# goroda/c3sc

Measured on AMD Instinct MI355X. Metric: Bellman-sweep nodes/sec (7D car rank-10), higher is better.
Workload: dtype f64

## Files before the change

### c3sc_amd/csrc/c3sc_hip.hip

```cpp
#include <hip/hip_runtime.h>

#include <algorithm>
#include <cmath>
#include <cstdio>
#include <cstdlib>
#include <cstring>
#include <string>
#include <vector>

#include "../../include/c3sc_hip.h"
#include "fiber_partition.hpp"
#include "kernel_common.hpp"
#include "kernel_rollout.hpp"
#include "kernel_rollout_ode.hpp"
#include "model_tables.hpp"
#include "registry.hpp"

namespace c3sc {

std::vector<KernelEntry> &kernel_registry()
{
    static std::vector<KernelEntry> reg;
    return reg;
}
// ... 715 lines not shown
    const int d = c->d;
    std::vector<int> rps(nstack);
    std::vector<long> offs((size_t)nstack * MAXD, 0);
    size_t off = c->static_doubles;
    for (int s = 0; s < nstack; s++) {
        const size_t *r = ranks + (size_t)s * (d + 1);
        if (r[0] != 1 || r[d] != 1) return fail(c, C3SC_ERR_ARG, "upload_value_stack: ranks[s][0] and ranks[s][d] must be 1");
        size_t maxrank = 1;
        for (int m = 0; m <= d; m++) {
            if (r[m] < 1) return fail(c, C3SC_ERR_ARG, "upload_value_stack: rank < 1");
            maxrank = std::max(maxrank, r[m]);
        }
        for (int m = 0; m < d; m++)
            if (!cores[(size_t)s * d + m]) return fail(c, C3SC_ERR_ARG, "upload_value_stack: null core");
        rps[s] = pick_rp(d, (int)maxrank, c->model, C3SC_VARIANT_AUTO);
        if (rps[s] == 0) return fail(c, C3SC_ERR_UNSUPPORTED, "upload_value_stack: no kernel instantiation for a stage's (dim, rank)");
        for (int m = 0; m < d; m++) {
            offs[(size_t)s * MAXD + m] = (long)off;
            const size_t per = (m == 0 || m == d - 1) ? rps[s] : (size_t)rps[s] * rps[s];
            off += ((size_t)c->ngrid[m] * per + 15) & ~(size_t)15;
        }
    }
    std::vector<double> buf(off - c->static_doubles, 0.0);
    for (int s = 0; s < nstack; s++) {
        double *dst[MAXD];
        for (int m = 0; m < d; m++) dst[m] = buf.data() + (offs[(size_t)s * MAXD + m] - (long)c->static_doubles);
        pad_cores_host(d, c->ngrid, rps[s], ranks + (size_t)s * (d + 1), cores + (size_t)s * d, dst);
    }
    HIPCHK(c, hipSetDevice(c->device));
    if (c->hz_stack) HIPCHK(c, hipFree(c->hz_stack));
    c->hz_stack = nullptr;
    c->hz_nstack = 0;
    HIPCHK(c, hipMalloc((void **)&c->hz_stack, off * sizeof(double)));
    HIPCHK(c, hipMemcpy(c->hz_stack + c->static_doubles, buf.data(), buf.size() * sizeof(double), hipMemcpyHostToDevice));
    c->hz_stack_static = c->static_doubles;
    c->hz_rp.swap(rps);
    c->hz_core_off.swap(offs);
    c->hz_nstack = nstack;
    return C3SC_OK;
}

int c3sc_hip_upload_value_device(c3sc_hip_ctx *c, const size_t *ranks, const double *const *d_cores, void *stream)
{
    size_t cd = 0;
    int rc = prepare_value(c, ranks, &cd);
    if (rc != C3SC_OK) return rc;
    const int d = c->d, rp = c->rp;
    for (int m = 0; m < d; m++) {
        const int kind = (m == 0) ? 0 : (m == d - 1 ? 2 : 1);
        const long total = (long)c->ngrid[m] * (kind == 1 ? rp * rp : rp);
        const int grid = (int)std::min<long>((total + 255) / 256, 1024);
        hipLaunchKernelGGL(k_pad_core, dim3(grid), dim3(256), 0, (hipStream_t)stream, d_cores[m], c->arena + c->core_off[m],
                           c->ngrid[m], (int)ranks[m], (int)ranks[m + 1], rp, kind);
    }
    HIPCHK(c, hipGetLastError());
    rc = make_quad_aux(c, stream);
    if (rc != C3SC_OK) return rc;
    c->have_value = true;
    return C3SC_OK;
}

static int fill_args(c3sc_hip_ctx *c, int k, size_t F, KArgs &A, bool need_model)
{
    if (!c) return C3SC_ERR_ARG;
    if (c->d == 0 || !c->have_boundary || !c->have_value) return fail(c, C3SC_ERR_ARG, "launch: grid, boundary and value must be set");
    if (need_model && (!c->have_mca || c->model == 0 || c->ncand == 0))
        return fail(c, C3SC_ERR_ARG, "launch: mca, model and controls must be set");
    if (k < 0 || k >= c->d) return fail(c, C3SC_ERR_ARG, "launch: dim_vary out of range");
    HIPCHK(c, hipSetDevice(c->device));
    if (c->static_dirty) {
        if (static_layout(c) != c->static_doubles)
            return fail(c, C3SC_ERR_ARG, "launch: static data changed size after upload_value; upload the value again");
        int rc = upload_static(c);
        if (rc != C3SC_OK) return rc;
    }
    std::memset(&A, 0, sizeof(A));
    A.d = c->d;
    A.k = k;
    A.N = c->ngrid[k];
    A.ncand = c->ncand;
    A.F = (long)F;
    for (int m = 0; m < c->d; m++) {
        A.ngrid[m] = c->ngrid[m];
        A.bctype[m] = c->bctype[m];
        A.xg_off[m] = c->xg_off_rel[m];
        A.core_off[m] = c->core_off[m];
        A.quad_coreT_off[m] = c->coreT_off[m];
        A.quad_aop_off[m] = c->aop_off[m];
        A.pair_img_off[m] = c->img_off[m];
        A.quad_imgL_off[m] = c->qimgL_off[m];
        A.quad_imgR_off[m] = c->qimgR_off[m];
    }
    A.img_base = c->arena;
    if (c->tabL_off && (c->tabL_off != pair_tabL_off(A, c->rp) || c->tabR_off != pair_tabR_off(A, c->rp)))
        return fail(c, C3SC_ERR_ARG, "launch: the pair kernel's product tables are not where the kernel looks for them");
    A.cends = c->cends;
    A.memo_keys = nullptr;
    A.skip = c->skip_flag;
    A.nobs = c->nobs;
    A.obs_off = c->obs_off;
    A.cands_off = c->cands_off;
    for (int t = 0; t < 4; t++) A.tab_off[t] = c->tab_off[t];
    A.cfeat_off = c->cfeat_off;
    A.h2 = c->h2;
    A.discount = c->discount;
    for (int i = 0; i < 2 * c->d; i++) A.t[i] = c->t[i];
    for (int i = 0; i < C3SC_MAX_PARAMS; i++) A.prm[i] = c->prm[i];
    A.status = c->d_status;
    A.game_gsz = c->game_gsz;
    A.game_ngrp = c->game_ngrp;
    A.game_order = c->game_order;
    A.hz_off = c->hz_dt > 0.0 ? c->hz_off : 0;
    {
        static const int dbg_env = [] { const char *e = getenv("C3SC_DBG"); return e ? atoi(e) : 0; }();
        A.dbg = dbg_env;
        if (dbg_env && !c->d_dbg) { HIPCHK(c, hipMalloc((void **)&c->d_dbg, 65536 * 8 * sizeof(unsigned long long))); }
        A.dbgbuf = c->d_dbg;
        if (A.dbg & 8) A.ncand = 1;
        if (A.dbg & 16) A.ncand = 3;
    }
    return C3SC_OK;
}

static void arm_memo(c3sc_hip_ctx *c, const KernelEntry *e, KArgs &A)
{
    A.memo_keys = nullptr;
    if (c->memo.keys == nullptr || e->variant != C3SC_VARIANT_FIBER_PER_WAVE) return;
    A.memo_keys = c->memo.keys; A.memo_vals = c->memo.vals; A.memo_capmask = c->memo.capmask; A.memo_epoch_bits = c->memo.epoch_bits;
    A.memo_shift = c->memo.shift; A.memo_counters = c->memo.counters; A.memo_mode = c->memo.mode;
    for (int m = 0; m < c->d; m++) A.memo_stride[m] = c->memo.stride[m];
    c->memo.applied = true;
}

static int launch_one(c3sc_hip_ctx *c, const KernelEntry *e, const KArgs &A, const LaunchIO &io, const char *unsupported = nullptr)
{
    c->last_kernel = e->name;
    g_launches++;
    c->status_cache_valid = false;
    const hipError_t he = launch_entry(*e, A, io);
    if (he == hipErrorNotSupported && unsupported) return fail(c, C3SC_ERR_UNSUPPORTED, unsupported);
    HIPCHK(c, he);
    return C3SC_OK;
}

constexpr long FIBER_PARTITION_MIN = 524288;
static long fiber_partition_min()
{
    const char *e = getenv("C3SC_FIBER_PARTITION");
    if (!e || !*e) return FIBER_PARTITION_MIN;
    const long v = atol(e);
    return v > 0 ? v : -1;
}

static int partition_fibers(c3sc_hip_ctx *c, const KernelEntry *e, const KArgs &A, LaunchIO &io, int slot, int &launched)
{
    io.perm = nullptr;
    io.nlive = nullptr;
    launched = 0;
    if (e->variant != C3SC_VARIANT_FIBER_PAIR || e->rtc || A.ncand > 64) return C3SC_OK;
    bool faces = false;
    for (int m = 0; m < A.d; m++) faces = faces || (m != A.k && A.bctype[m] == C3SC_ABSORB);
    const long fmin = fiber_partition_min();
    if (!faces || fmin < 0 || A.F < fmin || A.F > 0x40000000L) return C3SC_OK;
    const size_t need = fpart_bytes(A.F);
    if (need > c->part_bytes[slot]) {
        if (c->part[slot]) HIPCHK(c, hipFree(c->part[slot]));
        c->part[slot] = nullptr;
        c->part_bytes[slot] = 0;
        HIPCHK(c, hipMalloc(&c->part[slot], need));
        c->part_bytes[slot] = need;
    }
    const PartScratch ps = fpart_carve(c->part[slot], A.F);
    PartArgs P;
    P.d = A.d;
    P.k = A.k;
    P.F = A.F;
    for (int m = 0; m < MAXD; m++) { P.ngrid[m] = A.ngrid[m]; P.bctype[m] = A.bctype[m]; }
    HIPCHK(c, fpart_launch(P, io.idx, ps, io.stream));
    launched = 3;
    io.perm = ps.perm;
    io.nlive = ps.nlive;
    return C3SC_OK;
}

static int launch_bellman(c3sc_hip_ctx *c, int k, size_t F, const int32_t *d_idx, const int32_t *d_policy, double *d_out,
                          int32_t *d_uidx, int32_t *d_absorbed, void *stream, int part_slot = 0)
{
    KArgs A;
    int rc = fill_args(c, k, F, A, true);
    if (rc != C3SC_OK) return rc;
    int variant = c->variant;
    if (c->game_gsz > 0) {
        rc = check_game_model(c, "bellman_fibers: game mode needs a model compiled with game kernels of the game's du");
        if (rc != C3SC_OK) return rc;
        if (variant != C3SC_VARIANT_AUTO && variant != C3SC_VARIANT_FIBER_PER_WAVE)
            return fail(c, C3SC_ERR_UNSUPPORTED, "bellman_fibers: game mode runs on the fiber-per-wave kernel only (the pair and quad variants have no game form)");
        variant = C3SC_VARIANT_FIBER_PER_WAVE;
    }
    if (c->hz_dt > 0.0) {
        rc = check_horizon_model(c, "bellman_fibers: horizon mode needs a model compiled with horizon kernels (and no game)");
        if (rc != C3SC_OK) return rc;
        if (variant != C3SC_VARIANT_AUTO && variant != C3SC_VARIANT_FIBER_PER_WAVE)
            return fail(c, C3SC_ERR_UNSUPPORTED, "bellman_fibers: horizon mode runs on the fiber-per-wave kernel only (the pair and quad variants have no horizon form)");
        variant = C3SC_VARIANT_FIBER_PER_WAVE;
    }
    if (F == 0) return C3SC_OK;
    if (!d_idx || !d_out) return fail(c, C3SC_ERR_ARG, "bellman_fibers: null buffer");
    A.forced = d_policy;
    LaunchIO io{c->arena, d_idx, d_out, d_uidx, d_absorbed, nullptr, nullptr, nullptr, nullptr, (hipStream_t)stream};
    std::vector<const KernelEntry *> declined;
    hipError_t he = hipSuccess;
    int part_launches = 0;
    for (;;) {
        const KernelEntry *e = find_kernel(c->model, c->d, c->rp, A.N, variant, k, F, &declined);
        if (!e || e->rp != c->rp) {
            if (declined.empty()) return fail(c, C3SC_ERR_UNSUPPORTED, "bellman_fibers: no kernel instantiation for (model, dim, rank, N)");
            return fail(c, C3SC_ERR_UNSUPPORTED, he == hipErrorOutOfMemory
                            ? "bellman_fibers: N x rank^2 of the varying core exceeds the 160 KB of LDS the per-wave kernel stages it in"
                            : "bellman_fibers: no kernel instantiation serves this call (model, dim, rank, N, control mode)");
        }
        c->last_kernel = e->name;
        arm_memo(c, e, A);
        rc = partition_fibers(c, e, A, io, part_slot, part_launches);
        if (rc != C3SC_OK) return rc;
        he = launch_entry(*e, A, io);
        if (he != hipErrorOutOfMemory && he != hipErrorNotSupported) break;
        c->memo.applied = false;
        if (getenv("C3SC_VERBOSE")) fprintf(stderr, "c3sc: %s declined (%s), trying the next instantiation\n", e->name, hipGetErrorName(he));
        declined.push_back(e);
    }
    g_launches += 1 + part_launches;
    c->status_cache_valid = false;
    HIPCHK(c, he);
    return C3SC_OK;
}

int c3sc_hip_bellman_fibers(c3sc_hip_ctx *c, int k, size_t F, const int32_t *d_idx, double *d_out, int32_t *d_uidx,
                            int32_t *d_absorbed, void *stream)
{
    return launch_bellman(c, k, F, d_idx, nullptr, d_out, d_uidx, d_absorbed, stream);
}

static int launch_bellman_all(c3sc_hip_ctx *c, int nk, const int *ks, const size_t *F, const int32_t *const *d_idx,
                              const int32_t *const *d_policy, double *const *d_out, int32_t *const *d_uidx, int32_t *const *d_absorbed,
                              void *stream)
{
    if (!c) return C3SC_ERR_ARG;
    if (nk < 1 || nk > MAXD || !ks || !F || !d_idx || !d_out) return fail(c, C3SC_ERR_ARG, "bellman_fibers_all: bad arguments");
    static const bool no_overlap = getenv("C3SC_NO_OVERLAP") != nullptr;
    bool overlap = nk > 1 && !no_overlap && c->memo.keys == nullptr && c->skip_flag == nullptr;
    for (int s = 0; s < nk; s++) {
        if (ks[s] < 0 || ks[s] >= c->d) return fail(c, C3SC_ERR_ARG, "bellman_fibers_all: dim_vary out of range");
        if (F[s] > 0 && (!d_idx[s] || !d_out[s])) return fail(c, C3SC_ERR_ARG, "bellman_fibers_all: null buffer");
        if (d_policy && !d_policy[s]) return fail(c, C3SC_ERR_ARG, "bellman_fibers_all: null policy");
        for (int q = 0; q < s; q++)
            if (d_out[q] == d_out[s] && F[s] > 0) return fail(c, C3SC_ERR_ARG, "bellman_fibers_all: two segments share an output array");
    }
    hipStream_t st = (hipStream_t)stream;
    if (overlap) {
        HIPCHK(c, hipSetDevice(c->device));
        if (!c->fork_ev) {
            HIPCHK(c, hipEventCreateWithFlags(&c->fork_ev, hipEventDisableTiming));
            for (int i = 0; i < c3sc_hip_ctx::NSIDE; i++) {
                HIPCHK(c, hipStreamCreateWithFlags(&c->side[i], hipStreamNonBlocking));
                HIPCHK(c, hipEventCreateWithFlags(&c->join_ev[i], hipEventDisableTiming));
            }
        }
        HIPCHK(c, hipEventRecord(c->fork_ev, st));
        for (int i = 0; i < c3sc_hip_ctx::NSIDE; i++) HIPCHK(c, hipStreamWaitEvent(c->side[i], c->fork_ev, 0));
    }
    int rc = C3SC_OK;
    for (int s = 0; s < nk && rc == C3SC_OK; s++) {
        const int lane = overlap ? s % (c3sc_hip_ctx::NSIDE + 1) : 0;
        rc = launch_bellman(c, ks[s], F[s], d_idx[s], d_policy ? d_policy[s] : nullptr, d_out[s], d_uidx ? d_uidx[s] : nullptr,
                            d_absorbed ? d_absorbed[s] : nullptr, lane == 0 ? stream : (void *)c->side[lane - 1], lane);
    }
    if (overlap)
        for (int i = 0; i < c3sc_hip_ctx::NSIDE; i++) {
            HIPCHK(c, hipEventRecord(c->join_ev[i], c->side[i]));
            HIPCHK(c, hipStreamWaitEvent(st, c->join_ev[i], 0));
        }
    return rc;
}

int c3sc_hip_bellman_fibers_all(c3sc_hip_ctx *c, int nk, const int *ks, const size_t *F, const int32_t *const *d_idx, double *const *d_out,
                                int32_t *const *d_uidx, int32_t *const *d_absorbed, void *stream)
{
    return launch_bellman_all(c, nk, ks, F, d_idx, nullptr, d_out, d_uidx, d_absorbed, stream);
}

int c3sc_hip_policy_fibers_all(c3sc_hip_ctx *c, int nk, const int *ks, const size_t *F, const int32_t *const *d_idx,
                               const int32_t *const *d_policy, double *const *d_out, int32_t *const *d_absorbed, void *stream)
{
    if (!d_policy) return fail(c, C3SC_ERR_ARG, "policy_fibers_all: null policy");
    return launch_bellman_all(c, nk, ks, F, d_idx, d_policy, d_out, nullptr, d_absorbed, stream);
}

static int launch_box(c3sc_hip_ctx *c, int k, size_t F, const int32_t *d_idx, const double *d_policy_u, double *d_out,
                      double *d_uopt, int32_t *d_absorbed, void *stream)
{
    if (!c) return C3SC_ERR_ARG;
    if (c->box_du == 0) return fail(c, C3SC_ERR_ARG, "bellman_fibers_box: c3sc_hip_set_control_box first");
    if (c->game_gsz > 0) return fail(c, C3SC_ERR_UNSUPPORTED, "bellman_fibers_box: games have no control-box form");
    if (c->hz_dt > 0.0) return fail(c, C3SC_ERR_UNSUPPORTED, "bellman_fibers_box: horizon mode has no control-box form");
    if (model_ncf(c->model) != 0 && c->model != C3SC_MODEL_COTHRUST6D)
        return fail(c, C3SC_ERR_UNSUPPORTED, "bellman_fibers_box: this model needs transcendental functions of the control");
    KArgs A;
    int rc = fill_args(c, k, F, A, true);
    if (rc != C3SC_OK) return rc;
    if (F == 0) return C3SC_OK;
    if (!d_idx || !d_out) return fail(c, C3SC_ERR_ARG, "bellman_fibers_box: null buffer");
    A.cmode = 1;
    A.ugrid = c->box_grid;
    A.upolish = c->box_polish;
    for (int i = 0; i < c->box_du; i++) { A.ulb[i] = c->box_lb[i]; A.uub[i] = c->box_ub[i]; }
    A.uopt = d_uopt;
    A.forced_u = d_policy_u;
    const KernelEntry *e = find_kernel(c->model, c->d, c->rp, A.N, C3SC_VARIANT_FIBER_PER_WAVE, k);
    if (!e || e->rp != c->rp) return fail(c, C3SC_ERR_UNSUPPORTED, "bellman_fibers_box: no fiber-per-wave instantiation for (model, dim, rank, N)");
    arm_memo(c, e, A);
    LaunchIO io{c->arena, d_idx, d_out, nullptr, d_absorbed, nullptr, nullptr, nullptr, nullptr, (hipStream_t)stream};
    return launch_one(c, e, A, io, "bellman_fibers_box: no box-minimiser instantiation for this model");
}

int c3sc_hip_bellman_fibers_box(c3sc_hip_ctx *c, int k, size_t F, const int32_t *d_idx, double *d_out, double *d_uopt,
                                int32_t *d_absorbed, void *stream)
{
    return launch_box(c, k, F, d_idx, nullptr, d_out, d_uopt, d_absorbed, stream);
}

// ... 392 lines not shown

int c3sc_hip_simulate_host(c3sc_hip_ctx *c, const c3sc_hip_sim_args *h)
{
    if (!c) return C3SC_ERR_ARG;
    if (!h) return fail(c, C3SC_ERR_ARG, "simulate_host: null argument struct");
    if (h->n == 0) return c3sc_hip_simulate(c, h, nullptr);
    HostShape sh;
    const int rc = closed_loop_host_shape(c, "simulate", h, h->nsteps, sh);
    if (rc != C3SC_OK) return rc;
    const size_t n = sh.n, d = sh.d, D = sizeof(double);
    return stage_host(c, STAGE_PER_CALL, "simulate_host",
                      {{h->d_x0, n * d * D, SEG_IN}, {h->d_noise, h->d_noise ? n * h->nsteps * d * D : 0, SEG_IN},
                       {h->d_traj, h->d_traj ? n * sh.nrow * d * D : 0, SEG_OUT}, {h->d_u, h->d_u ? n * sh.nurow * sh.du * D : 0, SEG_OUT},
                       {h->d_cost, n * D, SEG_OUT}, {h->d_exit, n * sizeof(int64_t), SEG_OUT}, {h->d_vend, n * D, SEG_OUT},
                       {h->d_xfinal, n * d * D, SEG_OUT}},
                      [&](const DevPtr *b) {
                          c3sc_hip_sim_args a = *h;
                          a.d_x0 = b[0]; a.d_noise = b[1]; a.d_traj = b[2]; a.d_u = b[3];
                          a.d_cost = b[4]; a.d_exit = b[5]; a.d_vend = b[6]; a.d_xfinal = b[7];
                          return c3sc_hip_simulate(c, &a, nullptr);
                      });
}

static const size_t ODE_MAX_EVALS = (size_t)1 << 40;

static long long ode_nsub(double dt_out, double dt_int)
{
    if (dt_int == 0.0) return 1;
    const double r = dt_out / dt_int, q = std::nearbyint(r);
    if (!(q >= 1.0) || !(std::fabs(r - q) <= 1e-9 * q) || q > (double)(1 << 30)) return 0;
    return (long long)q;
}

static bool ode_box_ok(const double *b, int d)
{
    if (!b) return true;
    for (int m = 0; m < d; m++)
        if (!(b[m] <= b[d + m])) return false;
    return true;
}

int c3sc_hip_integrate(c3sc_hip_ctx *c, const c3sc_hip_ode_args *a, void *stream)
{
    const char *who = "integrate";
    int rc = closed_loop_setup(c, who, a);
    if (rc != C3SC_OK) return rc;
    if (c->hz_dt > 0.0) return fail(c, C3SC_ERR_UNSUPPORTED, "integrate: deterministic closed loops are not offered in horizon mode");
    KArgs A;
    rc = fill_args(c, 0, 0, A, false);
    if (rc != C3SC_OK) return rc;
    rc = check_bounds_set(c, "integrate: every dimension needs a boundary type");
    if (rc != C3SC_OK) return rc;
    if (!(a->dt_out > 0.0) || !std::isfinite(a->dt_out)) return fail(c, C3SC_ERR_ARG, "integrate: dt_out must be positive and finite");
    if (!(a->dt_int >= 0.0) || !std::isfinite(a->dt_int)) return fail(c, C3SC_ERR_ARG, "integrate: dt_int must be >= 0 and finite");
    const long long nsub = ode_nsub(a->dt_out, a->dt_int);
    if (nsub == 0) return fail(c, C3SC_ERR_ARG, "integrate: dt_out / dt_int is not an integer (to 1e-9 relative)");
    if (a->method != C3SC_ODE_FORWARD_EULER && a->method != C3SC_ODE_RK4)
        return fail(c, C3SC_ERR_ARG, "integrate: method must be C3SC_ODE_FORWARD_EULER or C3SC_ODE_RK4");
    const int nstage = a->method == C3SC_ODE_RK4 ? 4 : 1;
    if (a->nout > (size_t)1 << 30) return fail(c, C3SC_ERR_ARG, "integrate: nout too large");
    if ((size_t)nsub * a->nout * nstage > ODE_MAX_EVALS) return fail(c, C3SC_ERR_ARG, "integrate: more than 2^40 controller evaluations per trajectory");
    rc = closed_loop_sizes(c, who, a, a->nout, "integrate: more than 2^31 trajectories in one call (split the batch)",
                           "integrate: save_every larger than nout");
    if (rc != C3SC_OK) return rc;
    if (a->evals_per_launch < 0) return fail(c, C3SC_ERR_ARG, "integrate: evals_per_launch < 0");
    if (!ode_box_ok(a->goal, c->d) || !ode_box_ok(a->keep, c->d))
        return fail(c, C3SC_ERR_ARG, "integrate: a stop box has lo > hi (or a NaN)");
    const KernelEntry *e = find_sim_kernel(VARIANT_ROLLOUT_ODE, c->model, c->d, c->rp);
    if (!e) return fail(c, C3SC_ERR_UNSUPPORTED, "integrate: no integrate instantiation for this model at this padded rank");
    if (a->n == 0) return C3SC_OK;
    if (!a->d_x0) return fail(c, C3SC_ERR_ARG, "integrate: null d_x0");
    const int d = c->d;
    const size_t n = a->n;
    rc = closed_loop_state(c, n * (size_t)(d + 3) * sizeof(double));
    if (rc != C3SC_OK) return rc;
    closed_loop_box(c, a->box, A);
    OdeK S;
    std::memset(&S, 0, sizeof(S));
    S.n = (long)n;
    S.nsub = (int)nsub;
    S.nout = (int)a->nout;
    S.nstage = nstage;
    S.save_every = (int)a->save_every;
    S.wrap = a->wrap_periodic ? 1 : 0;
    S.constelm = c->constelm;
    S.h = a->dt_int == 0.0 ? a->dt_out : a->dt_int;
    S.dt_out = a->dt_out;
    S.has_goal = a->goal ? 1 : 0;
    S.has_keep = a->keep ? 1 : 0;
    for (int m = 0; m < d; m++) {
        S.goal_lo[m] = a->goal ? a->goal[m] : 0.0;
        S.goal_hi[m] = a->goal ? a->goal[d + m] : 0.0;
        S.keep_lo[m] = a->keep ? a->keep[m] : -INFINITY;
        S.keep_hi[m] = a->keep ? a->keep[d + m] : INFINITY;
    }
    S.x0 = a->d_x0;
    S.x = (double *)c->sim_state;
    S.cost = S.x + n * d;
    S.stop_step = (long long *)(S.cost + n);
    S.stop_reason = (int32_t *)(S.stop_step + n);
    S.traj = a->d_traj;
    S.u = a->d_u;
    S.vend = a->d_vend;
    const long long ktot = nsub * (long long)a->nout;
    const long long chunk = std::max<long long>(1, (a->evals_per_launch > 0 ? a->evals_per_launch : 256) / nstage);
    long long k0 = 0;
    do {
        S.k0 = k0;
        S.k1 = std::min(k0 + chunk, ktot);
        LaunchIO io{c->arena, nullptr, nullptr, nullptr, nullptr, nullptr, nullptr, nullptr, nullptr, (hipStream_t)stream, &S};
        rc = launch_one(c, e, A, io, "integrate: this integrate kernel has no box minimiser");
        if (rc != C3SC_OK) return rc;
        k0 = S.k1;
    } while (k0 < ktot);
    rc = closed_loop_results(c, a, a->d_stop_step, stream);
    if (rc != C3SC_OK) return rc;
    return copy_back(c, a->d_stop_reason, S.stop_reason, n * sizeof(int32_t), stream);
}

int c3sc_hip_integrate_host(c3sc_hip_ctx *c, const c3sc_hip_ode_args *h)
{
    if (!c) return C3SC_ERR_ARG;
    if (!h) return fail(c, C3SC_ERR_ARG, "integrate_host: null argument struct");
    if (h->n == 0) return c3sc_hip_integrate(c, h, nullptr);
    HostShape sh;
    const int rc = closed_loop_host_shape(c, "integrate", h, h->nout, sh);
    if (rc != C3SC_OK) return rc;
    const size_t n = sh.n, d = sh.d, D = sizeof(double);
    return stage_host(c, STAGE_PER_CALL, "integrate_host",
                      {{h->d_x0, n * d * D, SEG_IN}, {h->d_traj, h->d_traj ? n * sh.nrow * d * D : 0, SEG_OUT},
                       {h->d_u, h->d_u ? n * sh.nurow * sh.du * D : 0, SEG_OUT}, {h->d_cost, n * D, SEG_OUT},
                       {h->d_stop_step, n * sizeof(int64_t), SEG_OUT}, {h->d_stop_reason, n * sizeof(int32_t), SEG_OUT},
                       {h->d_vend, n * D, SEG_OUT}, {h->d_xfinal, n * d * D, SEG_OUT}},
                      [&](const DevPtr *b) {
                          c3sc_hip_ode_args a = *h;
                          a.d_x0 = b[0]; a.d_traj = b[1]; a.d_u = b[2]; a.d_cost = b[3];
                          a.d_stop_step = b[4]; a.d_stop_reason = b[5]; a.d_vend = b[6]; a.d_xfinal = b[7];
                          return c3sc_hip_integrate(c, &a, nullptr);
                      });
}

int c3sc_hip_normals(uint64_t seed, uint64_t traj0, size_t ntraj, uint64_t step0, size_t nsteps, int dw, double *out)
{
    if (!out || dw < 1 || dw > MAXD) return C3SC_ERR_ARG;
    for (size_t t = 0; t < ntraj; t++)
        for (size_t k = 0; k < nsteps; k++)
            for (int j = 0; j < dw; j++)
                out[(t * nsteps + k) * dw + j] = philox_normal(seed, traj0 + t, (uint32_t)(step0 + k), (uint32_t)j);
    return C3SC_OK;
}

unsigned long long c3sc_hip_launch_count(void) { return g_launches; }

int c3sc_hip_debug_read(c3sc_hip_ctx *c, unsigned long long *out, size_t n)
{
    if (!c || !c->d_dbg || !out) return C3SC_ERR_ARG;
    HIPCHK(c, hipMemcpy(out, c->d_dbg, n * sizeof(unsigned long long), hipMemcpyDeviceToHost));
    return C3SC_OK;
}

int c3sc_hip_timer_start(c3sc_hip_ctx *c, void *stream)
{
    if (!c) return C3SC_ERR_ARG;
    HIPCHK(c, hipEventRecord(c->ev0, (hipStream_t)stream));
    return C3SC_OK;
}

int c3sc_hip_timer_stop(c3sc_hip_ctx *c, void *stream, float *ms)
{
    if (!c || !ms) return C3SC_ERR_ARG;
    HIPCHK(c, hipEventRecord(c->ev1, (hipStream_t)stream));
    HIPCHK(c, hipEventSynchronize(c->ev1));
    HIPCHK(c, hipEventElapsedTime(ms, c->ev0, c->ev1));
    return C3SC_OK;
}

static int run_peak(c3sc_hip_ctx *c, bool mfma, double *tflops)
{
    if (!c || !tflops) return C3SC_ERR_ARG;
    HIPCHK(c, hipSetDevice(c->device));
    const char *ev = getenv("C3SC_PEAK_BLOCKS_PER_CU");
    const int blocks = 256 * (ev ? atoi(ev) : 8), threads = 256, iters = 20000;
    int rc = ensure_scratch(c, (size_t)blocks * threads * sizeof(double));
    if (rc != C3SC_OK) return rc;
    float best = 1e30f;
    for (int rep = 0; rep < 4; rep++) {
        HIPCHK(c, hipEventRecord(c->ev0, nullptr));
        if (mfma) hipLaunchKernelGGL(k_peak_mfma, dim3(blocks), dim3(threads), 0, nullptr, (double *)c->scratch, iters);
        else hipLaunchKernelGGL(k_peak_fma, dim3(blocks), dim3(threads), 0, nullptr, (double *)c->scratch, iters);
        HIPCHK(c, hipEventRecord(c->ev1, nullptr));
        HIPCHK(c, hipEventSynchronize(c->ev1));
        float ms = 0;
        HIPCHK(c, hipEventElapsedTime(&ms, c->ev0, c->ev1));
        if (rep > 0 && ms < best) best = ms;
    }
    const double waves = (double)blocks * threads / 64.0;
    const double flop = mfma ? waves * iters * 4.0 * (2.0 * 16 * 16 * 4) : (double)blocks * threads * iters * 8.0 * 2.0;
    *tflops = flop / (best * 1e-3) / 1e12;
    return C3SC_OK;
}

int c3sc_hip_peak_fma_f64(c3sc_hip_ctx *c, double *tflops) { return run_peak(c, false, tflops); }
int c3sc_hip_peak_mfma_f64(c3sc_hip_ctx *c, double *tflops) { return run_peak(c, true, tflops); }

}
```

### c3sc_amd/csrc/ctx.hpp

```cpp
#pragma once
#include <hip/hip_runtime.h>

#include <string>
#include <vector>

#include "../../include/c3sc_hip.h"
#include "kernel_common.hpp"

struct c3sc_cross_dev;
struct c3sc_hip_comm;

struct c3sc_hip_ctx {
    int device = 0;
    std::string err;
    int d = 0;
    int ngrid[c3sc::MAXD] = {0};
    std::vector<double> xgrid_flat;
    int xg_off_rel[c3sc::MAXD] = {0};
    int bctype[c3sc::MAXD] = {0};
    int cends = 0;
    bool have_boundary = false;
    int nobs = 0;
    std::vector<double> obs;
    bool have_mca = false;
    double h2 = 0, discount = 0, t[2 * c3sc::MAXD] = {0};
    int model = 0;
    double prm[C3SC_MAX_PARAMS] = {0};
    int ncand = 0, du = 0;
    std::vector<double> cands;
    int game_gsz = 0, game_ngrp = 0, game_order = 0;
    double hz_dt = 0.0;
    int hz_off = 0;
    double *hz_stack = nullptr;
    size_t hz_stack_static = 0;
    int hz_nstack = 0;
    std::vector<int> hz_rp;
    std::vector<long> hz_core_off;
    int box_du = 0, box_grid = 0, box_polish = 0;
    double box_lb[C3SC_MAX_DU] = {0}, box_ub[C3SC_MAX_DU] = {0};
    bool have_value = false;
    size_t ranks[c3sc::MAXD + 1] = {0};
    int rp = 0;
    double *arena = nullptr;
    size_t arena_cap = 0;
    size_t static_doubles = 0;
    bool static_dirty = true;
    long core_off[c3sc::MAXD] = {0};
    long coreT_off[c3sc::MAXD] = {0}, aop_off[c3sc::MAXD] = {0};
    long img_off[c3sc::MAXD] = {0};
    long qimgL_off[c3sc::MAXD] = {0}, qimgR_off[c3sc::MAXD] = {0};
    long tabL_off = 0, tabR_off = 0;
    int obs_off = 0, cands_off = 0, tab_off[4] = {0, 0, 0, 0}, cfeat_off = 0;
    unsigned *d_status = nullptr;
    unsigned status_cache = 0;
    bool status_cache_valid = false;
    unsigned long long *d_dbg = nullptr;
    int variant = C3SC_VARIANT_AUTO;
    const char *last_kernel = "";
    hipEvent_t ev0 = nullptr, ev1 = nullptr;
    static constexpr int NSIDE = 2;
    hipStream_t side[NSIDE] = {nullptr, nullptr};
    hipEvent_t fork_ev = nullptr, join_ev[NSIDE] = {nullptr, nullptr};
    void *part[NSIDE + 1] = {nullptr, nullptr, nullptr};
    size_t part_bytes[NSIDE + 1] = {0, 0, 0};
    void *scratch = nullptr;
    size_t scratch_bytes = 0;
    void *sim_state = nullptr;
    size_t sim_state_bytes = 0;
    int constelm = 0;
    void *pinned = nullptr, *pinned_dev = nullptr;
    size_t pinned_bytes = 0;
    struct {
        unsigned long long *keys = nullptr;
        double *vals = nullptr;
        unsigned long long capmask = 0, epoch_bits = 0;
        int shift = 0;
        long long stride[c3sc::MAXD] = {0};
        unsigned long long *counters = nullptr;
        int mode = 0;
        bool applied = false;
    } memo;
    const int *skip_flag = nullptr;
    c3sc_hip_comm *shard_comm = nullptr;
    c3sc_cross_dev *cross = nullptr;
};

#define HIPCHK(ctx, call)                                                                    \
    do {                                                                                     \
        hipError_t e__ = (call);                                                             \
        if (e__ != hipSuccess) {                                                             \
            (ctx)->err = std::string(#call) + ": " + hipGetErrorString(e__);                 \
            return C3SC_ERR_HIP;                                                             \
        }                                                                                    \
    } while (0)

static inline int fail(c3sc_hip_ctx *ctx, int code, const char *msg)
{
    if (ctx) ctx->err = msg;
    return code;
}
```

### c3sc_amd/csrc/fiber_partition.hpp

```cpp
#pragma once
#include <hip/hip_runtime.h>

#include "kernel_common.hpp"

namespace c3sc {

constexpr int FPART_THREADS = 256, FPART_PER_THREAD = 4, FPART_BLOCK = FPART_THREADS * FPART_PER_THREAD;

struct PartArgs {
    int d, k;
    long F;
    int ngrid[MAXD];
    int bctype[MAXD];
};

struct PartScratch {
    int32_t *perm = nullptr;
    int32_t *blocks = nullptr;
    int32_t *nlive = nullptr;
    uint8_t *flags = nullptr;
};

__host__ __device__ constexpr size_t fpart_align(size_t b) { return (b + 255) & ~(size_t)255; }
inline long fpart_blocks(long F) { return (F + FPART_BLOCK - 1) / FPART_BLOCK; }
inline size_t fpart_bytes(long F)
{
    return fpart_align((size_t)F * 4) + fpart_align((size_t)fpart_blocks(F) * 4) + fpart_align(4) + fpart_align((size_t)F);
}
inline PartScratch fpart_carve(void *base, long F)
{
    PartScratch s;
    char *p = (char *)base;
    s.perm = (int32_t *)p;
    p += fpart_align((size_t)F * 4);
    s.blocks = (int32_t *)p;
    p += fpart_align((size_t)fpart_blocks(F) * 4);
    s.nlive = (int32_t *)p;
    p += fpart_align(4);
    s.flags = (uint8_t *)p;
    return s;
}

__device__ inline bool fiber_dead(const PartArgs &P, const int32_t *__restrict__ idx, long f)
{
    bool dead = false;
    for (int m = 0; m < P.d; m++) {
        if (m == P.k) continue;
        int lo, hi;
        dead = fixed_neighbors(idx[f * P.d + m], P.ngrid[m], P.bctype[m], lo, hi) || dead;
    }
    return dead;
}

__device__ inline int fpart_block_scan(int v, int &total)
{
    __shared__ int wsum[FPART_THREADS / 64];
    const int lane = threadIdx.x & 63, w = threadIdx.x >> 6;
    int inc = v;
#pragma unroll
    for (int o = 1; o < 64; o <<= 1) {
        const int t = __shfl_up(inc, o, 64);
        if (lane >= o) inc += t;
    }
    __syncthreads();
    if (lane == 63) wsum[w] = inc;
    __syncthreads();
    int before = 0;
    total = 0;
#pragma unroll
    for (int q = 0; q < FPART_THREADS / 64; q++) {
        if (q < w) before += wsum[q];
        total += wsum[q];
    }
    return before + inc - v;
}

__global__ void __launch_bounds__(FPART_THREADS) k_fpart_count(const PartArgs P, const int32_t *__restrict__ idx, uint8_t *__restrict__ flags,
                                                               int32_t *__restrict__ blocks)
{
    const long f0 = (long)blockIdx.x * FPART_BLOCK + (long)threadIdx.x * FPART_PER_THREAD;
    int live = 0;
#pragma unroll
    for (int i = 0; i < FPART_PER_THREAD; i++) {
        const long f = f0 + i;
        if (f < P.F) {
            const bool dead = fiber_dead(P, idx, f);
            flags[f] = dead ? 1 : 0;
            live += dead ? 0 : 1;
        }
    }
    int total;
    (void)fpart_block_scan(live, total);
    if (threadIdx.x == 0) blocks[blockIdx.x] = total;
}

__global__ void __launch_bounds__(FPART_THREADS) k_fpart_scan(int32_t *__restrict__ blocks, long nblocks, int32_t *__restrict__ nlive)
{
    int carry = 0;
    for (long b0 = 0; b0 < nblocks; b0 += FPART_THREADS) {
        const long b = b0 + threadIdx.x;
        const int v = b < nblocks ? blocks[b] : 0;
        int total;
        const int ex = fpart_block_scan(v, total);
        if (b < nblocks) blocks[b] = carry + ex;
        carry += total;
    }
    if (threadIdx.x == 0) *nlive = carry;
}

__global__ void __launch_bounds__(FPART_THREADS) k_fpart_scatter(long F, const uint8_t *__restrict__ flags, const int32_t *__restrict__ blocks,
                                                                 const int32_t *__restrict__ nlive, int32_t *__restrict__ perm)
{
    const long fb = (long)blockIdx.x * FPART_BLOCK, f0 = fb + (long)threadIdx.x * FPART_PER_THREAD;
    bool dead[FPART_PER_THREAD];
    int live = 0;
#pragma unroll
    for (int i = 0; i < FPART_PER_THREAD; i++) {
        dead[i] = (f0 + i < F) ? flags[f0 + i] != 0 : true;
        live += dead[i] ? 0 : 1;
    }
    int total;
    const int ex = fpart_block_scan(live, total);
    const long live_before = blocks[blockIdx.x];
    long lpos = live_before + ex;
    long dpos = (long)*nlive + (fb - live_before) + ((long)threadIdx.x * FPART_PER_THREAD - ex);
#pragma unroll
    for (int i = 0; i < FPART_PER_THREAD; i++) {
        if (f0 + i < F) {
            if (dead[i]) perm[dpos++] = (int32_t)(f0 + i);
            else perm[lpos++] = (int32_t)(f0 + i);
        }
    }
}

inline hipError_t fpart_launch(const PartArgs &P, const int32_t *idx, const PartScratch &s, hipStream_t stream)
{
    const long nb = fpart_blocks(P.F);
    hipLaunchKernelGGL(k_fpart_count, dim3((unsigned)nb), dim3(FPART_THREADS), 0, stream, P, idx, s.flags, s.blocks);
    hipLaunchKernelGGL(k_fpart_scan, dim3(1), dim3(FPART_THREADS), 0, stream, s.blocks, nb, s.nlive);
    hipLaunchKernelGGL(k_fpart_scatter, dim3((unsigned)nb), dim3(FPART_THREADS), 0, stream, P.F, (const uint8_t *)s.flags, (const int32_t *)s.blocks,
                       (const int32_t *)s.nlive, s.perm);
    return hipGetLastError();
}

}
```

### c3sc_amd/csrc/fold_lds.hpp

```cpp
#pragma once
#include <utility>

#include "kernel_common.hpp"

namespace c3sc {

#ifndef FPL_NV
#define FPL_NV 2
#endif
#ifndef FPL_NO_FENCE
#define FPL_SCHED_FENCE() asm volatile("" ::: "memory")
#else
#define FPL_SCHED_FENCE()
#endif

__host__ __device__ constexpr int fpl_lds_stride(int elems) { return elems | 1; }

__device__ __forceinline__ void pin(double &x) { asm volatile("" : "+v"(x)); }
__device__ __forceinline__ void mem_fence() { asm volatile("" ::: "memory"); }

template <int RP, int NV>
__device__ inline void vecmat_lds(const double *G, double (&v)[NV][RP])
{
    double t[NV][RP];
    double g[2][RP];
#pragma unroll
    for (int s = 0; s < NV; s++)
#pragma unroll
        for (int b = 0; b < RP; b++) t[s][b] = 0.0;
#pragma unroll
    for (int b = 0; b < RP; b++) g[0][b] = G[b * RP];
#pragma unroll
    for (int a = 0; a < RP; a++) {
        if (a + 1 < RP) {
#pragma unroll
            for (int b = 0; b < RP; b++) g[(a + 1) & 1][b] = G[(a + 1) + b * RP];
        }
#pragma unroll
        for (int s = 0; s < NV; s++)
#pragma unroll
            for (int b = 0; b < RP; b++) {
                t[s][b] = fma(v[s][a], g[a & 1][b], t[s][b]);
                pin(t[s][b]);
            }
        mem_fence();
    }
#pragma unroll
    for (int s = 0; s < NV; s++)
#pragma unroll
        for (int b = 0; b < RP; b++) v[s][b] = t[s][b];
}

template <int RP, int NV>
__device__ inline void matvec_lds(const double *G, double (&v)[NV][RP])
{
    double t[NV][RP];
    double g[2][RP];
#pragma unroll
    for (int s = 0; s < NV; s++)
#pragma unroll
        for (int a = 0; a < RP; a++) t[s][a] = 0.0;
#pragma unroll
    for (int a = 0; a < RP; a++) g[0][a] = G[a];
#pragma unroll
    for (int b = 0; b < RP; b++) {
        if (b + 1 < RP) {
#pragma unroll
            for (int a = 0; a < RP; a++) g[(b + 1) & 1][a] = G[a + (b + 1) * RP];
        }
#pragma unroll
        for (int s = 0; s < NV; s++)
#pragma unroll
            for (int a = 0; a < RP; a++) {
                t[s][a] = fma(g[b & 1][a], v[s][b], t[s][a]);
                pin(t[s][a]);
            }
        mem_fence();
    }
#pragma unroll
    for (int s = 0; s < NV; s++)
#pragma unroll
        for (int a = 0; a < RP; a++) v[s][a] = t[s][a];
}

template <int RP, int NW, int FIRST, int COUNT, bool ROWVEC, int NVMAX = FPL_NV>
__device__ inline void apply_core(const double *G, double (&W)[NW][RP])
{
    if constexpr (COUNT > 0) {
        constexpr int NV = COUNT >= NVMAX ? NVMAX : COUNT;
        double tmp[NV][RP];
#pragma unroll
        for (int s = 0; s < NV; s++)
#pragma unroll
            for (int a = 0; a < RP; a++) tmp[s][a] = W[FIRST + s][a];
        if constexpr (ROWVEC) vecmat_lds<RP, NV>(G, tmp);
        else matvec_lds<RP, NV>(G, tmp);
#pragma unroll
        for (int s = 0; s < NV; s++)
#pragma unroll
            for (int a = 0; a < RP; a++) W[FIRST + s][a] = tmp[s][a];
        apply_core<RP, NW, FIRST + NV, COUNT - NV, ROWVEC, NVMAX>(G, W);
    }
}

template <int RP>
__device__ inline double dot_reg(const double (&a)[RP], const double (&b)[RP])
{
    double s = 0.0;
#pragma unroll
    for (int i = 0; i < RP; i++) s = fma(a[i], b[i], s);
    return s;
}

template <int RP, int NV, bool ROWVEC>
__device__ __forceinline__ void apply_glb(const double *__restrict__ G, double (&v)[NV][RP])
{
    constexpr int CH = (RP <= 4) ? RP : (RP <= 6 ? 3 : 2);
    double t[NV][RP];
#pragma unroll
    for (int s = 0; s < NV; s++)
#pragma unroll
        for (int i = 0; i < RP; i++) t[s][i] = 0.0;
#pragma unroll
    for (int b0 = 0; b0 < RP; b0 += CH) {
        int off = b0 * RP;
        asm volatile("" : "+v"(off));
        const double *Gc = G + off;
        double g[CH][RP];
#pragma unroll
        for (int b = 0; b < CH; b++)
#pragma unroll
            for (int a = 0; a < RP; a++) g[b][a] = (b0 + b < RP) ? Gc[a + b * RP] : 0.0;
#pragma unroll
        for (int b = 0; b < CH; b++) {
            if (b0 + b < RP) {
#pragma unroll
                for (int s = 0; s < NV; s++)
#pragma unroll
                    for (int a = 0; a < RP; a++) {
                        if constexpr (ROWVEC) t[s][b0 + b] = fma(v[s][a], g[b][a], t[s][b0 + b]);
                        else t[s][a] = fma(g[b][a], v[s][b0 + b], t[s][a]);
                    }
            }
        }
#pragma unroll
        for (int s = 0; s < NV; s++)
#pragma unroll
            for (int i = 0; i < RP; i++) pin(t[s][i]);
    }
#pragma unroll
    for (int s = 0; s < NV; s++)
#pragma unroll
        for (int i = 0; i < RP; i++) v[s][i] = t[s][i];
}

template <int RP, int NW, int FIRST, int COUNT, bool ROWVEC>
__device__ __forceinline__ void apply_range_glb(const double *__restrict__ G, double (&W)[NW][RP])
{
    if constexpr (COUNT > 0) {
        constexpr int NV = COUNT >= 2 ? 2 : 1;
        double tmp[NV][RP];
#pragma unroll
        for (int s = 0; s < NV; s++)
#pragma unroll
            for (int a = 0; a < RP; a++) tmp[s][a] = W[FIRST + s][a];
        apply_glb<RP, NV, ROWVEC>(G, tmp);
#pragma unroll
        for (int s = 0; s < NV; s++)
#pragma unroll
            for (int a = 0; a < RP; a++) W[FIRST + s][a] = tmp[s][a];
        apply_range_glb<RP, NW, FIRST + NV, COUNT - NV, ROWVEC>(G, W);
    }
}

__device__ inline void dimk_values(int jn, int N, int bck, double vL, double vC, double vR, double vwrap, double vone,
                                   double &lo, double &hi)
{
    lo = vL;
    hi = vR;
    if (jn == 0) {
        lo = (bck == C3SC_PERIODIC) ? vwrap : vC;
        hi = (bck == C3SC_ABSORB) ? vC : vR;
    }
    if (jn == N - 1) {
        lo = (bck == C3SC_ABSORB) ? vC : vL;
        hi = (bck == C3SC_PERIODIC) ? vone : vC;
        if (N == 1) lo = vC;
    }
}

}
```

### c3sc_amd/csrc/kernel_common.hpp

```cpp
#pragma once
#ifdef __HIPCC_RTC__
#include "rtc_prelude.hpp"
#else
#include <type_traits>
#include <hip/hip_runtime.h>
#include <stdint.h>
#endif

#include "../../include/c3sc_hip.h"

#ifdef C3SC_STAMPS
#define C3SC_STAMPS_ON 1
#else
#define C3SC_STAMPS_ON 0
#endif

namespace c3sc {

constexpr int MAXD = C3SC_MAX_DIM;

struct KArgs {
    int d, k, N, ncand;
    long F;
    int ngrid[MAXD];
    int bctype[MAXD];
    int xg_off[MAXD];
    long core_off[MAXD];
    int nobs;
    int obs_off;
    int cands_off;
    int tab_off[4];
    int cfeat_off;
    double h2, discount;
    double t[2 * MAXD];
    double prm[C3SC_MAX_PARAMS];
    unsigned *status;
    unsigned long long *dbgbuf;
    const int32_t *forced;
    int dbg;
    int cmode, ugrid, upolish;
    double ulb[C3SC_MAX_DU], uub[C3SC_MAX_DU];
    double *uopt;
    const double *forced_u;
    int tbl_off;
    int hz_off;
    long quad_coreT_off[MAXD];
    long quad_aop_off[MAXD];
    int quad_sv_off;
    int quad_x_off;
    int quad_m1_off;
    int quad_ix_off;
    long quad_imgL_off[MAXD];
    long quad_imgR_off[MAXD];
    long pair_img_off[MAXD];
    int cends;
    int game_gsz;
    unsigned long long *memo_keys;
    double *memo_vals;
    unsigned long long memo_capmask, memo_epoch_bits;
    int memo_shift;
    int game_ngrp;
    long long memo_stride[MAXD];
    unsigned long long *memo_counters;
    const int *skip;
    int memo_mode;
    int game_order;
    const double *img_base;
};

__host__ __device__ constexpr long arena_block(long doubles) { return (doubles + 15) & ~15L; }
__host__ __device__ constexpr long pair_img_doubles(int nodes, int per) { return arena_block((long)nodes * (per | 1) + 2); }
__host__ __device__ constexpr long pair_tab_doubles(int na, int nb, int rp) { return arena_block((long)na * nb * rp); }
__host__ __device__ inline long pair_tabL_off(const KArgs &A, int rp) { return A.pair_img_off[A.d - 1] + pair_img_doubles(A.ngrid[A.d - 1], rp); }
__host__ __device__ inline long pair_tabR_off(const KArgs &A, int rp) { return pair_tabL_off(A, rp) + pair_tab_doubles(A.ngrid[0], A.ngrid[1], rp); }

__device__ inline int game_list_to_pair(const KArgs &A, int p)
{
    return A.game_order == C3SC_GAME_MAXMIN ? (p % A.game_gsz) * A.game_ngrp + p / A.game_gsz : p;
}
__device__ inline int game_pair_to_list(const KArgs &A, int i)
{
    return A.game_order == C3SC_GAME_MAXMIN ? (i % A.game_ngrp) * A.game_gsz + i / A.game_ngrp : i;
}

template <class M>
struct GameOf : M {
    static constexpr bool GAME = true;
};
template <class Model>
constexpr bool model_game()
{
    if constexpr (requires { Model::GAME; }) return Model::GAME;
    else return false;
}

template <class M>
struct HorizonOf : M {
    static constexpr bool HORIZON = true;
};
template <class Model>
constexpr bool model_horizon()
{
    if constexpr (requires { Model::HORIZON; }) return Model::HORIZON;
    else return false;
}

struct KOut {
    double *out;
    double *costs;
    int32_t *uidx;
    int32_t *absorbed;
};

__device__ inline void wave_sync()
{
    __builtin_amdgcn_fence(__ATOMIC_RELEASE, "wavefront");
    __builtin_amdgcn_wave_barrier();
    __builtin_amdgcn_fence(__ATOMIC_ACQUIRE, "wavefront");
}

__device__ inline bool fixed_neighbors(int i, int n, int bc, int &lo, int &hi)
{
    const bool first = (i == 0), last = (i == n - 1) & !first;
    const bool absorb = (bc == C3SC_ABSORB), reflect = (bc == C3SC_REFLECT);
    const int lo_first = absorb ? i : (reflect ? i : n - 2);
    const int hi_first = absorb ? i : i + 1;
    const int lo_last = absorb ? i : i - 1;
    const int hi_last = absorb ? i : (reflect ? i : 1);
    lo = first ? lo_first : (last ? lo_last : i - 1);
    hi = first ? hi_first : (last ? hi_last : i + 1);
    return (first | last) & absorb;
}

__device__ inline int vary_neighbors(int j, int n, int bc, int ab_in, int &lo, int &hi, int keep_ends = 0)
{
    int ab = ab_in;
    const int ab_end = keep_ends ? ab_in : 0;
    if (j == 0) {
        if (bc == C3SC_ABSORB) { lo = 0; hi = 0; ab = 1; }
        else if (bc == C3SC_REFLECT) { lo = 0; hi = 1; ab = ab_end; }
        else { lo = n - 2; hi = 1; ab = ab_end; }
    } else if (j == n - 1) {
        if (bc == C3SC_ABSORB) { lo = n - 1; hi = n - 1; ab = 1; }
        else if (bc == C3SC_REFLECT) { lo = n - 2; hi = n - 1; ab = ab_end; }
        else { lo = n - 2; hi = 1; ab = ab_end; }
    } else if (ab == 0) {
        lo = j - 1;
        hi = j + 1;
    } else {
        lo = j;
        hi = j;
    }
    return ab;
}

constexpr unsigned long long MEMO_PENDING = 1ull << 48, MEMO_EPOCH_MASK = ~((1ull << 49) - 1), MEMO_ID_MASK = (1ull << 48) - 1;
__device__ inline double memo_merge(unsigned long long *keys, double *vals, unsigned long long capmask, int shift, unsigned long long epoch_bits,
                                    unsigned long long id, double v, int &inserted, int &overflow)
{
    const unsigned long long K = epoch_bits | id, KP = K | MEMO_PENDING;
    unsigned long long slot = (id * 0x9E3779B97F4A7C15ull) >> shift;
    for (unsigned long long probe = 0; probe <= capmask; probe++, slot = (slot + 1) & capmask) {
        unsigned long long cur = __hip_atomic_load(&keys[slot], __ATOMIC_ACQUIRE, __HIP_MEMORY_SCOPE_AGENT);
        while ((cur & MEMO_EPOCH_MASK) != epoch_bits) {
            const unsigned long long prev = atomicCAS(&keys[slot], cur, KP);
            if (prev == cur) {
                vals[slot] = v;
                __hip_atomic_store(&keys[slot], K, __ATOMIC_RELEASE, __HIP_MEMORY_SCOPE_AGENT);
                inserted = 1;
                return v;
            }
            cur = prev;
        }
        if ((cur & ~MEMO_PENDING) == K)
            return (cur & MEMO_PENDING) ? v : __hip_atomic_load(&vals[slot], __ATOMIC_RELAXED, __HIP_MEMORY_SCOPE_AGENT);
    }
    overflow = 1;
    return v;
}

template <int D>
__device__ inline bool in_obstacle(const KArgs &A, const double *__restrict__ ro, const double (&x)[D])
{
    int any = 0;
    for (int o = 0; o < A.nobs; o++) {
        const double *lb = ro + A.obs_off + (size_t)o * 2 * D;
        const double *ub = lb + D;
        int outside = 0;
#pragma unroll
        for (int m = 0; m < D; m++) outside |= (int)(x[m] < lb[m]) | (int)(x[m] > ub[m]);
        any |= (outside == 0);
    }
    return any != 0;
}

template <int D>
__device__ inline unsigned obstacle_mask_fixed(const KArgs &A, const double *__restrict__ ro, const double (&x)[D], int skip)
{
    unsigned mask = 0;
    for (int o = 0; o < A.nobs; o++) {
        const double *lb = ro + A.obs_off + (size_t)o * 2 * D;
        const double *ub = lb + D;
        int outside = 0;
#pragma unroll
        for (int m = 0; m < D; m++)
            if (m != skip) outside |= (int)(x[m] < lb[m]) | (int)(x[m] > ub[m]);
        mask |= (outside == 0 ? 1u : 0u) << o;
    }
    return mask;
}
template <int D>
__device__ inline unsigned obstacle_mask_dim(const KArgs &A, const double *__restrict__ ro, int k, double xk)
{
    unsigned mask = 0;
    for (int o = 0; o < A.nobs; o++) {
        const double lb = ro[A.obs_off + (size_t)o * 2 * D + k], ub = ro[A.obs_off + (size_t)o * 2 * D + D + k];
        mask |= ((xk < lb || xk > ub) ? 0u : 1u) << o;
    }
    return mask;
}

__device__ __forceinline__ void pin_vgpr(double &x) { asm volatile("" : "+v"(x)); }

__device__ __forceinline__ double readlane_f64(double v, int lane)
{
    const long long b = __double_as_longlong(v);
    const int lo = __builtin_amdgcn_readlane((int)(b & 0xffffffffll), lane);
    const int hi = __builtin_amdgcn_readlane((int)(b >> 32), lane);
// ... 758 lines not shown
```

### c3sc_amd/csrc/kernel_fiber_pair.hpp

```cpp
#pragma once
#include <utility>

#include "fold_lds.hpp"

#ifndef FPP_CGD
#define FPP_CGD 3
#endif
#ifndef FPP_PIPE2
#define FPP_PIPE2 1
#endif
#ifndef FPP_CG
#define FPP_CG 1
#endif
#ifndef FPP_NV
#define FPP_NV 4
#endif

#ifndef FPP_DIRECT_MAXD
#define FPP_DIRECT_MAXD 3
#endif
#ifndef FPP_EDGE_TABLES
#define FPP_EDGE_TABLES 1
#endif

#ifndef FPP_NODE_SPLIT
#define FPP_NODE_SPLIT 1
#endif
#ifndef FPP_NODE_SPLIT_VGPRS
#define FPP_NODE_SPLIT_VGPRS 140
#endif

namespace c3sc {

constexpr int FPP_THREADS = 128;

template <class Model, int RP>
__host__ __device__ constexpr bool fpp_direct() { return Model::D <= FPP_DIRECT_MAXD && RP <= 8; }

template <class Model, int RP>
__host__ __device__ constexpr bool fpp_edge_tables() { return FPP_EDGE_TABLES && !fpp_direct<Model, RP>() && Model::D >= 4; }

template <int RP>
__device__ __forceinline__ void load_row16(const double *__restrict__ p, double (&r)[RP])
{
    typedef double v2d __attribute__((ext_vector_type(2)));
#pragma unroll
    for (int i = 0; i < RP / 2; i++) {
        const v2d v = *reinterpret_cast<const v2d *>(p + 2 * i);
        r[2 * i] = v.x;
        r[2 * i + 1] = v.y;
    }
}

template <int RP, int NW, int FIRST, int COUNT, bool ROWVEC>
__device__ inline void apply_core_and(const double *G, double (&W)[NW][RP], double (&E)[RP])
{
    constexpr int N1 = COUNT >= FPP_NV - 1 ? FPP_NV - 1 : COUNT;
    double tmp[N1 + 1][RP];
#pragma unroll
    for (int a = 0; a < RP; a++) tmp[0][a] = E[a];
#pragma unroll
    for (int s = 0; s < N1; s++)
#pragma unroll
        for (int a = 0; a < RP; a++) tmp[s + 1][a] = W[FIRST + s][a];
    if constexpr (ROWVEC) vecmat_lds<RP, N1 + 1>(G, tmp);
    else matvec_lds<RP, N1 + 1>(G, tmp);
#pragma unroll
    for (int a = 0; a < RP; a++) E[a] = tmp[0][a];
#pragma unroll
    for (int s = 0; s < N1; s++)
#pragma unroll
        for (int a = 0; a < RP; a++) W[FIRST + s][a] = tmp[s + 1][a];
    apply_core<RP, NW, FIRST + N1, COUNT - N1, ROWVEC, FPP_NV>(G, W);
}

__device__ inline void pair_barrier()
{
    asm volatile("s_waitcnt lgkmcnt(0)\n\ts_barrier" ::: "memory");
}

template <int H>
__device__ inline void stage_core_image(double *sK, const double *img, int n_doubles)
{
    typedef __attribute__((address_space(3))) char lds_char;
    typedef __attribute__((address_space(3))) void lds_void;
    typedef const __attribute__((address_space(1))) void glb_void;
    const int pieces = (n_doubles + 1) >> 1;
    const int lane = threadIdx.x & 63;
    for (int base = H * 64; base < pieces; base += FPP_THREADS) {
        const int b = max(min(base, pieces - 64), 0);
        const int p = min(b + lane, pieces - 1);
        __builtin_amdgcn_global_load_lds((glb_void *)(img + 2 * p), (lds_void *)((lds_char *)sK + 16 * b), 16, 0, 0);
    }
    asm volatile("s_waitcnt vmcnt(0)" ::: "memory");
}

template <int K>
__host__ __device__ constexpr int pair_owner(int m) { return m < K ? ((K - 1 - m) & 1) : ((m - K) & 1); }

template <class Model, int K>
struct PairPark {
    static constexpr int D = Model::D, NTAB = Model::NTAB;
    static constexpr unsigned UM = Model::UDEP_MASK, UC = Model::UCONST_MASK, ALL = (1u << D) - 1u;
    __host__ __device__ static constexpr bool has_deps()
    {
        if constexpr (requires { Model::HAS_DEPS; }) return Model::HAS_DEPS;
        else return false;
    }
    __host__ __device__ static constexpr unsigned dep(int m)
    {
        if constexpr (has_deps()) return Model::dep_mask(m);
        else return ALL;
    }
    __host__ __device__ static constexpr unsigned cost_dep()
    {
        if constexpr (has_deps()) return Model::COST_DEP;
        else return ALL;
    }
    __host__ __device__ static constexpr unsigned constd()
    {
        unsigned c = 0;
        if (has_deps())
            for (int m = 0; m < D; m++)
                if (!((UM >> m) & 1u) && !((dep(m) >> K) & 1u)) c |= 1u << m;
        return c;
    }
    __host__ __device__ static constexpr unsigned need()
    {
        unsigned n = cost_dep();
        for (int m = 0; m < D; m++) {
            const bool ctl = (UM >> m) & 1u, cst = (constd() >> m) & 1u;
            if ((!ctl && !cst) || (ctl && !((UC >> m) & 1u))) n |= dep(m);
        }
        return n & ALL;
    }
    __host__ __device__ static constexpr bool need_x(int m) { return m != K && ((need() >> m) & 1u); }
    __host__ __device__ static constexpr bool need_t(int t) { return Model::tab_dim(t) != K && ((need() >> Model::tab_dim(t)) & 1u); }
    __host__ __device__ static constexpr int row_x(int m)
    {
        int r = 0;
        for (int q = 0; q < m; q++) r += need_x(q);
        return r;
    }
    __host__ __device__ static constexpr int nx() { return row_x(D); }
    __host__ __device__ static constexpr int row_t(int t)
    {
        int r = nx();
        for (int q = 0; q < t; q++) r += need_t(q);
        return r;
    }
    __host__ __device__ static constexpr int nt() { return row_t(NTAB) - nx(); }
    __host__ __device__ static constexpr unsigned merged() { return constd() & ~(1u << K); }
    __host__ __device__ static constexpr unsigned rates() { return constd() & (1u << K); }
    __host__ __device__ static constexpr int row_pm(int m)
    {
        int r = nx() + nt();
        for (int q = 0; q < m; q++) r += 2 * ((rates() >> q) & 1u);
        return r;
    }
    __host__ __device__ static constexpr int row_q() { return row_pm(D); }
    __host__ __device__ static constexpr int rows() { return row_q() + (merged() != 0u); }
};

struct FoldPlan {
    int lfirst, rfirst;
    bool ledge, redge;
    int staged;
    int products;
};
template <class Model, int K, bool TAB = false>
struct PairMap {
    typedef PairPark<Model, K> PK;
    static constexpr int D = Model::D, NIT = D + 2, UL = D, UR = D + 1;
    __host__ __device__ static constexpr bool ltab() { return TAB && K >= 2; }
    __host__ __device__ static constexpr bool rtab() { return TAB && K <= D - 3; }
    __host__ __device__ static constexpr bool mg(int m) { return (PK::merged() >> m) & 1u; }
    __host__ __device__ static constexpr int first_l()
    {
        for (int m = 0; m < K; m++)
            if (mg(m)) return m;
        return -1;
    }
    __host__ __device__ static constexpr int first_r()
    {
        for (int m = D - 1; m > K; m--)
            if (mg(m)) return m;
        return -1;
    }
    __host__ __device__ static constexpr bool valid(int it)
    {
        return it == UL ? first_l() >= 0 : (it == UR ? first_r() >= 0 : (it != K && !mg(it)));
    }
    __host__ __device__ static constexpr int count(int it) { return !valid(it) ? 0 : (it < D ? 2 : 1); }
    __host__ __device__ static constexpr int nvl()
    {
        int c = count(UL);
        for (int m = 0; m < K; m++) c += count(m);
        return c;
    }
    __host__ __device__ static constexpr int nvr()
    {
        int c = count(UR);
        for (int m = K + 1; m < D; m++) c += count(m);
        return c;
    }
    __host__ __device__ static constexpr int nv() { return nvl() + nvr(); }
    __host__ __device__ static constexpr int gslot(int it)
    {
        if (it == UL) return 0;
        if (it == UR) return nvl();
        int c = it < K ? count(UL) : nvl() + count(UR);
        for (int m = it < K ? 0 : K + 1; m < it; m++) c += count(m);
        return c;
    }
    __host__ __device__ static constexpr int cost(int it)
    {
        if (!valid(it)) return 0;
        constexpr int lf = ltab() ? 2 : 1, rf = rtab() ? D - 3 : D - 2;
        if (it == UL) {
            int c = K - 1 - first_l() - (ltab() && first_l() == 0);
            for (int m = lf; m < K; m++) c += 2 * mg(m);
            return c;
        }
        if (it == UR) {
            int c = first_r() - K - 1 - (rtab() && first_r() == D - 1);
            for (int m = K + 1; m <= rf; m++) c += 2 * mg(m);
            return c;
        }
        if (it < K) return (ltab() && it <= 1) ? 2 * (K - 2) : (it > 0 ? 2 : 0) + 2 * (K - 1 - it);
        return (rtab() && it >= D - 2) ? 2 * (D - 3 - K) : (it < D - 1 ? 2 : 0) + 2 * (it - K - 1);
    }
    __host__ __device__ static constexpr FoldPlan plan()
    {
        FoldPlan p{ltab() ? 2 : 1, rtab() ? D - 3 : D - 2, K > 0 && !TAB, K < D - 1 && !TAB, 0, 0};
        const int ls = K - p.lfirst > 0 ? K - p.lfirst : 0, rs = p.rfirst - K > 0 ? p.rfirst - K : 0;
        p.staged = ls + rs + p.ledge + p.redge;
        p.products = ls + rs;
        for (int it = 0; it < NIT; it++) p.products += cost(it);
        return p;
    }
    __host__ __device__ static constexpr int owner(int it)
    {
        if (PK::merged() == 0u) return pair_owner<K>(it);
        int load[2] = {0, 0}, own[NIT] = {};
        bool done[NIT] = {};
        for (int n = 0; n < NIT; n++) {
            int best = -1;
            for (int q = 0; q < NIT; q++)
                if (valid(q) && !done[q] && (best < 0 || cost(q) > cost(best))) best = q;
            if (best < 0) break;
            const int h = load[1] < load[0] ? 1 : 0;
            own[best] = h;
            load[h] += cost(best);
            done[best] = true;
        }
        return own[it];
    }
    __host__ __device__ static constexpr int created(int m)
    {
        if (m == K) return -1;
        if (!mg(m)) return m;
        return m < K ? (m == first_l() ? UL : -1) : (m == first_r() ? UR : -1);
    }
    template <int H>
    __host__ __device__ static constexpr int left_before(int m)
    {
        int c = 0;
        for (int q = 0; q < m && q < K; q++)
            if (created(q) >= 0 && owner(created(q)) == H) c += count(created(q));
        return c;
    }
    template <int H>
    __host__ __device__ static constexpr int right_after(int m)
    {
        int c = 0;
        for (int q = D - 1; q > m && q > K; q--)
            if (created(q) >= 0 && owner(created(q)) == H) c += count(created(q));
        return c;
    }
    template <int H>
    __host__ __device__ static constexpr int lslot(int it)
    {
        if (it == UL) return left_before<H>(first_l());
        if (it == UR) return left_before<H>(K) + right_after<H>(first_r());
        return it < K ? left_before<H>(it) : left_before<H>(K) + right_after<H>(it);
    }
};

__host__ __device__ constexpr bool fpp_node_split_optout(int d, int rp, int k) { return rp < 10 || (d == 7 && rp == 10 && k == 4); }
template <class Model, int RP, int K>
__host__ __device__ constexpr bool fpp_node_split()
{
    if constexpr (!FPP_NODE_SPLIT || fpp_direct<Model, RP>()) return false;
    else
        return PairPark<Model, K>::merged() != 0u && PairMap<Model, K>::nv() * RP * 2 <= FPP_NODE_SPLIT_VGPRS &&
               !fpp_node_split_optout(Model::D, RP, K);
}

template <class Model, int K>
struct PairPre {
    static constexpr unsigned MASK = PairPark<Model, K>::merged(), RATES = PairPark<Model, K>::rates();
    const double *PX;
    int lane;
    double pvc;
    __device__ inline double q() const { return PX[PairPark<Model, K>::row_q() * 64 + lane]; }
    __device__ inline double pv() const { return pvc; }
    __device__ inline double pm(int m) const { return PX[PairPark<Model, K>::row_pm(m) * 64 + lane]; }
    __device__ inline double pp(int m) const { return PX[(PairPark<Model, K>::row_pm(m) + 1) * 64 + lane]; }
};

#define FPP_STAMP(slot)                                                   \
    if (C3SC_STAMPS_ON && (A.dbg & 128)) {                                \
        const unsigned long long now__ = clock64();                       \
        seg[slot] += now__ - tlast;                                       \
        tlast = now__;                                                    \
    }

template <class Model, int RP, int K, int H, bool FORCED, bool PART>
__device__ __attribute__((always_inline)) inline void fiber_pair_body(const KArgs &A, const double *__restrict__ ro,
                                                                     const int32_t *__restrict__ idx, double *__restrict__ outv,
                                                                     int32_t *__restrict__ uidx, int32_t *__restrict__ absorbed,
                                                                     const int32_t *__restrict__ perm, const int32_t *__restrict__ nlive_p,
                                                                     double *sK, unsigned &st)
{
    constexpr int D = Model::D;
    constexpr int S = 2 * D + 1;
    constexpr int RH = RP / 2;
    typedef PairPark<Model, K> PK;
    constexpr bool ET = fpp_edge_tables<Model, RP>();
    typedef PairMap<Model, K, ET> PM;
    constexpr FoldPlan PL = PM::plan();
    constexpr int NV = PM::nv();
    constexpr int NVL = PM::nvl();
    constexpr int NOL = PM::template left_before<H>(K);
    constexpr int NOR = PM::template right_after<H>(K);
    constexpr int NOWN = (NOL + NOR) > 0 ? (NOL + NOR) : 1;
    constexpr int NP = NV + 1;
    constexpr bool DIRECT = fpp_direct<Model, RP>();
    static_assert(RP % 2 == 0, "rank-split kernel needs an even padded rank");
    const int lane = threadIdx.x & 63;
    const int N = A.N;
    const long ntiles = (A.F + 63) / 64;
    int first_dead = 0x7fffffff;
    if constexpr (PART) first_dead = __builtin_amdgcn_readfirstlane((int)(((long)*nlive_p + 63) >> 6));
    unsigned long long seg[12] = {0, 0, 0, 0, 0, 0, 0, 0, 0, 0, 0, 0}, tlast = clock64();
    CandLds<Model> cr;
    NodeLds<Model, K> nr;
    {
        CandRegs<Model> cr0;
        cr0.load(A, ro);
        NodeRegs<Model, K> nr0;
        nr0.load(A, ro);
        double *tb = sK + A.tbl_off;
        cr.fill(tb, cr0, A.ncand);
        nr.fill(tb + CandLds<Model>::doubles(A.ncand), nr0, N);
        pair_barrier();
    }

    for (long tile = blockIdx.x; tile < ntiles; tile += gridDim.x) {
        FPP_STAMP(7)
        const long f_raw = tile * 64 + lane;
        const bool live = f_raw < A.F;
        const long f_pos = live ? f_raw : A.F - 1;
        long f = f_pos;
        if constexpr (PART) f = (long)perm[f_pos];
        const bool dead_tile = PART && tile >= (long)first_dead;

        if constexpr (PART) if (dead_tile) {
            const bool whole = A.bctype[K] == C3SC_ABSORB || A.cends != 0;
            const int jb = whole ? 0 : 1, je = whole ? N : N - 1;
            double xb[D];
#pragma unroll
            for (int m = 0; m < D; m++) xb[m] = (m != K && PK::need_x(m)) ? ro[A.xg_off[m] + idx[f * D + m]] : 0.0;
            for (int j = jb + ((jb ^ H) & 1); j < je; j += 2) {
                xb[K] = nr.x_at(j);
                outv[(size_t)f * N + j] = Model::boundcost(A.prm, xb);
                if (uidx) uidx[(size_t)f * N + j] = -1;
                if (absorbed) absorbed[(size_t)f * N + j] = 1;
            }
            if (whole) continue;
        }

        int fi[D], nbm[D], nbp[D];
        bool fiber_abs = false;
        double x[D];
#pragma unroll
        for (int m = 0; m < D; m++) {
            fi[m] = (m == K) ? 0 : idx[f * D + m];
            const bool face = fixed_neighbors(fi[m], A.ngrid[m], A.bctype[m], nbm[m], nbp[m]);
            if (m != K) fiber_abs = fiber_abs || face;
            x[m] = ro[A.xg_off[m] + fi[m]];
        }

        const unsigned obs_fixed = obstacle_mask_fixed<D>(A, ro, x, K);
        double tv[Model::NTAB > 0 ? Model::NTAB : 1];
        table_values<Model>(A, ro, fi, tv);

        double rpm[D], rpp[D];
#pragma unroll
        for (int m = 0; m < D; m++) { rpm[m] = 0.0; rpp[m] = 0.0; }
        if constexpr (PK::constd() != 0) {
            typename Model::Node nd0;
            Model::prep(A.prm, x, tv, nd0);
            double u0[Model::DU], cf0[Model::NCF > 0 ? Model::NCF : 1], b0[D], s0[D];
#pragma unroll
            for (int i = 0; i < Model::DU; i++) u0[i] = cr.get_u(i, 0);
            cf0[0] = 0.0;
#pragma unroll
            for (int i = 0; i < Model::NCF; i++) cf0[i] = cr.get_cf(i, 0);
            Model::drift(A.prm, nd0, x, u0, cf0, b0);
            Model::sigma(A.prm, x, u0, s0);
#pragma unroll
            for (int m = 0; m < D; m++)
                if ((PK::constd() >> m) & 1u) upwind_rates(A.t[2 * m], A.t[2 * m + 1], b0[m], s0[m], rpm[m], rpp[m]);
        }

        double L[RP], R[RP], W[NOWN][RP];
#pragma unroll
        for (int a = 0; a < RP; a++) { L[a] = (a == 0) ? 1.0 : 0.0; R[a] = (a == 0) ? 1.0 : 0.0; }

        FPP_STAMP(0)
        if (!(C3SC_STAMPS_ON && (A.dbg & 1))) {
        if constexpr (K > 0) {
            constexpr bool OWN0 = PM::ltab() && (PM::mg(0) ? PM::owner(PM::UL) == H : PM::owner(0) == H);
            constexpr bool OWN1 = PM::ltab() && (PM::mg(1) ? PM::owner(PM::UL) == H : PM::owner(1) == H);
            double t0m[OWN0 ? RP : 1], t0p[OWN0 ? RP : 1], t1m[OWN1 ? RP : 1], t1p[OWN1 ? RP : 1];
            if constexpr (PM::ltab()) {
                const double *T = ro + pair_tabL_off(A, RP);
                const int n1 = A.ngrid[1];
                load_row16<RP>(T + ((long)fi[0] * n1 + fi[1]) * RP, L);
                if constexpr (OWN0) {
                    load_row16<RP>(T + ((long)nbm[0] * n1 + fi[1]) * RP, t0m);
                    load_row16<RP>(T + ((long)nbp[0] * n1 + fi[1]) * RP, t0p);
                }
                if constexpr (OWN1) {
                    load_row16<RP>(T + ((long)fi[0] * n1 + nbm[1]) * RP, t1m);
                    load_row16<RP>(T + ((long)fi[0] * n1 + nbp[1]) * RP, t1p);
                }
                __builtin_amdgcn_sched_barrier(0);
            }
            auto left_combine = [&]() __attribute__((always_inline)) {
                if constexpr (OWN0) {
#pragma unroll
                    for (int b = 0; b < RP; b++) {
                        if constexpr (PM::mg(0)) W[0][b] = fma(rpp[0], t0p[b], rpm[0] * t0m[b]);
                        else { W[0][b] = t0m[b]; W[1][b] = t0p[b]; }
                    }
                }
                if constexpr (OWN1) {
                    constexpr int before = PM::template left_before<H>(1);
#pragma unroll
                    for (int b = 0; b < RP; b++) {
                        if constexpr (PM::mg(1)) {
                            constexpr int su = PM::template lslot<H>(PM::UL);
                            const double nw = fma(rpp[1], t1p[b], rpm[1] * t1m[b]);
                            W[su][b] = (1 == PM::first_l()) ? nw : W[su][b] + nw;
                        } else { W[before][b] = t1m[b]; W[before + 1][b] = t1p[b]; }
                    }
                }
            };
            if constexpr (PM::ltab() && K == PL.lfirst) left_combine();
            if constexpr (!PM::ltab()) {
                constexpr bool GLB = DIRECT || !PL.ledge;
                constexpr int str = GLB ? RP : fpl_lds_stride(RP);
                const double *src = sK;
                FPP_STAMP(1)
                if constexpr (GLB) src = ro + A.core_off[0];
                else {
                    pair_barrier();
                    stage_core_image<H>(sK, A.img_base + A.pair_img_off[0], A.ngrid[0] * str);
                    pair_barrier();
                }
                FPP_STAMP(7)
#pragma unroll
                for (int b = 0; b < RP; b++) {
                    L[b] = src[fi[0] * str + b];
                    if constexpr (PM::mg(0)) {
                        if constexpr (PM::owner(PM::UL) == H) W[0][b] = fma(rpp[0], src[nbp[0] * str + b], rpm[0] * src[nbm[0] * str + b]);
                    } else if constexpr (PM::owner(0) == H) {
                        W[0][b] = src[nbm[0] * str + b];
                        W[1][b] = src[nbp[0] * str + b];
                    }
                }
            }
            auto left_step = [&](auto mc) __attribute__((always_inline)) {
                constexpr int m = decltype(mc)::value;
                constexpr int str = DIRECT ? RP * RP : fpl_lds_stride(RP * RP);
                constexpr int before = PM::template left_before<H>(m);
                constexpr bool PAIR = !PM::mg(m) && PM::owner(m) == H, ACC = PM::mg(m) && PM::owner(PM::UL) == H;
                double nw[RP];
                const double *src = sK;
                FPP_STAMP(1)
                if constexpr (DIRECT) src = ro + A.core_off[m];
                else {
                    pair_barrier();
                    stage_core_image<H>(sK, A.img_base + A.pair_img_off[m], A.ngrid[m] * str);
                    pair_barrier();
                }
                if constexpr (PM::ltab() && m == PL.lfirst) left_combine();
                FPP_STAMP(7)
                const double *G = src + fi[m] * str;
                if constexpr (PAIR || ACC) {
                    double t0[1][RP], t1[1][RP];
#pragma unroll
                    for (int a = 0; a < RP; a++) { t0[0][a] = L[a]; t1[0][a] = L[a]; }
                    if constexpr (DIRECT) {
                        apply_glb<RP, 1, true>(src + nbm[m] * str, t0);
                        apply_glb<RP, 1, true>(src + nbp[m] * str, t1);
                    } else {
                        vecmat_lds<RP, 1>(src + nbm[m] * str, t0);
                        vecmat_lds<RP, 1>(src + nbp[m] * str, t1);
                    }
#pragma unroll
                    for (int a = 0; a < RP; a++) {
                        if constexpr (PAIR) { W[before][a] = t0[0][a]; W[before + 1][a] = t1[0][a]; }
                        else nw[a] = fma(rpp[m], t1[0][a], rpm[m] * t0[0][a]);
                    }
                }
                if constexpr (DIRECT) {
                    double tl[1][RP];
#pragma unroll
                    for (int a = 0; a < RP; a++) tl[0][a] = L[a];
                    apply_glb<RP, 1, true>(G, tl);
#pragma unroll
                    for (int a = 0; a < RP; a++) L[a] = tl[0][a];
                    apply_range_glb<RP, NOWN, 0, before, true>(G, W);
                } else
                    apply_core_and<RP, NOWN, 0, before, true>(G, W, L);
                if constexpr (ACC) {
                    constexpr int su = PM::template lslot<H>(PM::UL);
#pragma unroll
                    for (int a = 0; a < RP; a++) W[su][a] = (m == PM::first_l()) ? nw[a] : W[su][a] + nw[a];
                }
            };
            [&]<int... Ms>(std::integer_sequence<int, Ms...>) { (left_step(std::integral_constant<int, Ms + PL.lfirst>{}), ...); }
            (std::make_integer_sequence<int, (K > PL.lfirst ? K - PL.lfirst : 0)>{});
        }

        if constexpr (K < D - 1) {
            constexpr bool OWN0 = PM::rtab() && (PM::mg(D - 1) ? PM::owner(PM::UR) == H : PM::owner(D - 1) == H);
            constexpr bool OWN1 = PM::rtab() && (PM::mg(D - 2) ? PM::owner(PM::UR) == H : PM::owner(D - 2) == H);
            double t0m[OWN0 ? RP : 1], t0p[OWN0 ? RP : 1], t1m[OWN1 ? RP : 1], t1p[OWN1 ? RP : 1];
            if constexpr (PM::rtab()) {
                const double *T = ro + pair_tabR_off(A, RP);
                const int n1 = A.ngrid[D - 1];
                load_row16<RP>(T + ((long)fi[D - 2] * n1 + fi[D - 1]) * RP, R);
                if constexpr (OWN0) {
                    load_row16<RP>(T + ((long)fi[D - 2] * n1 + nbm[D - 1]) * RP, t0m);
                    load_row16<RP>(T + ((long)fi[D - 2] * n1 + nbp[D - 1]) * RP, t0p);
                }
                if constexpr (OWN1) {
                    load_row16<RP>(T + ((long)nbm[D - 2] * n1 + fi[D - 1]) * RP, t1m);
                    load_row16<RP>(T + ((long)nbp[D - 2] * n1 + fi[D - 1]) * RP, t1p);
                }
                __builtin_amdgcn_sched_barrier(0);
            }
            auto right_combine = [&]() __attribute__((always_inline)) {
                if constexpr (OWN0) {
#pragma unroll
                    for (int a = 0; a < RP; a++) {
                        if constexpr (PM::mg(D - 1)) W[NOL][a] = fma(rpp[D - 1], t0p[a], rpm[D - 1] * t0m[a]);
                        else { W[NOL][a] = t0m[a]; W[NOL + 1][a] = t0p[a]; }
                    }
                }
                if constexpr (OWN1) {
                    constexpr int after = PM::template right_after<H>(D - 2);
#pragma unroll
                    for (int a = 0; a < RP; a++) {
                        if constexpr (PM::mg(D - 2)) {
                            constexpr int su = PM::template lslot<H>(PM::UR);
                            const double nw = fma(rpp[D - 2], t1p[a], rpm[D - 2] * t1m[a]);
                            W[su][a] = (D - 2 == PM::first_r()) ? nw : W[su][a] + nw;
                        } else { W[NOL + after][a] = t1m[a]; W[NOL + after + 1][a] = t1p[a]; }
                    }
                }
            };
            if constexpr (PM::rtab() && K == PL.rfirst) right_combine();
            if constexpr (!PM::rtab()) {
                constexpr bool GLB = DIRECT || !PL.redge;
                constexpr int str = GLB ? RP : fpl_lds_stride(RP);
                const double *src = sK;
                FPP_STAMP(1)
                if constexpr (GLB) src = ro + A.core_off[D - 1];
                else {
                    pair_barrier();
                    stage_core_image<H>(sK, A.img_base + A.pair_img_off[D - 1], A.ngrid[D - 1] * str);
                    pair_barrier();
                }
                FPP_STAMP(7)
#pragma unroll
                for (int a = 0; a < RP; a++) {
                    R[a] = src[fi[D - 1] * str + a];
                    if constexpr (PM::mg(D - 1)) {
                        if constexpr (PM::owner(PM::UR) == H)
                            W[NOL][a] = fma(rpp[D - 1], src[nbp[D - 1] * str + a], rpm[D - 1] * src[nbm[D - 1] * str + a]);
                    } else if constexpr (PM::owner(D - 1) == H) {
                        W[NOL][a] = src[nbm[D - 1] * str + a];
                        W[NOL + 1][a] = src[nbp[D - 1] * str + a];
                    }
                }
            }
            auto right_step = [&](auto mc) __attribute__((always_inline)) {
                constexpr int m = decltype(mc)::value;
                constexpr int str = DIRECT ? RP * RP : fpl_lds_stride(RP * RP);
                constexpr int after = PM::template right_after<H>(m);
                constexpr bool PAIR = !PM::mg(m) && PM::owner(m) == H, ACC = PM::mg(m) && PM::owner(PM::UR) == H;
                double nw[RP];
                const double *src = sK;
                FPP_STAMP(1)
                if constexpr (DIRECT) src = ro + A.core_off[m];
                else {
                    pair_barrier();
                    stage_core_image<H>(sK, A.img_base + A.pair_img_off[m], A.ngrid[m] * str);
                    pair_barrier();
                }
                if constexpr (PM::rtab() && m == PL.rfirst) right_combine();
                FPP_STAMP(7)
                const double *G = src + fi[m] * str;
                if constexpr (PAIR || ACC) {
                    double t0[1][RP], t1[1][RP];
#pragma unroll
                    for (int a = 0; a < RP; a++) { t0[0][a] = R[a]; t1[0][a] = R[a]; }
                    if constexpr (DIRECT) {
                        apply_glb<RP, 1, false>(src + nbm[m] * str, t0);
                        apply_glb<RP, 1, false>(src + nbp[m] * str, t1);
                    } else {
                        matvec_lds<RP, 1>(src + nbm[m] * str, t0);
                        matvec_lds<RP, 1>(src + nbp[m] * str, t1);
                    }
#pragma unroll
                    for (int a = 0; a < RP; a++) {
                        if constexpr (PAIR) { W[NOL + after][a] = t0[0][a]; W[NOL + after + 1][a] = t1[0][a]; }
                        else nw[a] = fma(rpp[m], t1[0][a], rpm[m] * t0[0][a]);
                    }
                }
                if constexpr (DIRECT) {
                    double tr[1][RP];
#pragma unroll
                    for (int a = 0; a < RP; a++) tr[0][a] = R[a];
                    apply_glb<RP, 1, false>(G, tr);
#pragma unroll
                    for (int a = 0; a < RP; a++) R[a] = tr[0][a];
                    apply_range_glb<RP, NOWN, NOL, after, false>(G, W);
                } else
                    apply_core_and<RP, NOWN, NOL, after, false>(G, W, R);
                if constexpr (ACC) {
                    constexpr int su = PM::template lslot<H>(PM::UR);
#pragma unroll
                    for (int a = 0; a < RP; a++) W[su][a] = (m == PM::first_r()) ? nw[a] : W[su][a] + nw[a];
                }
            };
            [&]<int... Ms>(std::integer_sequence<int, Ms...>) { (right_step(std::integral_constant<int, PL.rfirst - Ms>{}), ...); }
            (std::make_integer_sequence<int, (PL.rfirst - K > 0 ? PL.rfirst - K : 0)>{});
        }

        }
        FPP_STAMP(1)
        constexpr bool NS = fpp_node_split<Model, RP, K>();
        double Wh[NS ? 1 : NV][RH];
        double Wf[NS ? NV : 1][RP];
        if constexpr (NS) {
            double *X = sK;
            auto put_get_own = [&](auto ic, auto pc) __attribute__((always_inline)) {
                constexpr int it = decltype(ic)::value, P = decltype(pc)::value;
                if constexpr (PM::valid(it) && PM::owner(it) == H) {
                    constexpr int slot = PM::template lslot<H>(it);
#pragma unroll
                    for (int s = 0; s < PM::count(it); s++) {
                        const int g = PM::gslot(it) + s;
#pragma unroll
                        for (int i = 0; i < RH; i++) {
                            X[(g * RH + i) * 64 + lane] = W[slot + s][P * RH + i];
                            Wf[g][P * RH + i] = W[slot + s][P * RH + i];
                        }
                    }
                }
            };
            auto get_other = [&](auto ic, auto pc) __attribute__((always_inline)) {
                constexpr int it = decltype(ic)::value, P = decltype(pc)::value;
                if constexpr (PM::valid(it) && PM::owner(it) != H) {
#pragma unroll
                    for (int s = 0; s < PM::count(it); s++) {
                        const int g = PM::gslot(it) + s;
#pragma unroll
                        for (int i = 0; i < RH; i++) Wf[g][P * RH + i] = X[(g * RH + i) * 64 + lane];
                    }
                }
            };
            auto half = [&](auto pc) __attribute__((always_inline)) {
                pair_barrier();
                [&]<int... Ms>(std::integer_sequence<int, Ms...>) { (put_get_own(std::integral_constant<int, Ms>{}, pc), ...); }
                (std::make_integer_sequence<int, PM::NIT>{});
                pair_barrier();
                [&]<int... Ms>(std::integer_sequence<int, Ms...>) { (get_other(std::integral_constant<int, Ms>{}, pc), ...); }
                (std::make_integer_sequence<int, PM::NIT>{});
            };
            half(std::integral_constant<int, 0>{});
            half(std::integral_constant<int, 1>{});
            pair_barrier();
        } else {
            double *X = sK;
            pair_barrier();
            auto put_get_own = [&](auto ic) __attribute__((always_inline)) {
                constexpr int it = decltype(ic)::value;
                if constexpr (PM::valid(it) && PM::owner(it) == H) {
                    constexpr int slot = PM::template lslot<H>(it);
#pragma unroll
                    for (int s = 0; s < PM::count(it); s++) {
                        const int g = PM::gslot(it) + s;
#pragma unroll
                        for (int i = 0; i < RH; i++) {
                            X[(g * RH + i) * 64 + lane] = W[slot + s][(1 - H) * RH + i];
                            Wh[g][i] = W[slot + s][H * RH + i];
                        }
                    }
                }
            };
            [&]<int... Ms>(std::integer_sequence<int, Ms...>) { (put_get_own(std::integral_constant<int, Ms>{}), ...); }
            (std::make_integer_sequence<int, PM::NIT>{});
            pair_barrier();
            auto get_other = [&](auto ic) __attribute__((always_inline)) {
                constexpr int it = decltype(ic)::value;
                if constexpr (PM::valid(it) && PM::owner(it) != H) {
#pragma unroll
                    for (int s = 0; s < PM::count(it); s++) {
                        const int g = PM::gslot(it) + s;
#pragma unroll
                        for (int i = 0; i < RH; i++) Wh[g][i] = X[(g * RH + i) * 64 + lane];
                    }
                }
            };
            [&]<int... Ms>(std::integer_sequence<int, Ms...>) { (get_other(std::integral_constant<int, Ms>{}), ...); }
            (std::make_integer_sequence<int, PM::NIT>{});
            pair_barrier();
        }
        double *sL = sK, *sR = sK + RP * 64;
        {
#pragma unroll
            for (int a = 0; a < RP; a++) {
                if constexpr (H == 0) sL[a * 64 + lane] = L[a];
                else sR[a * 64 + lane] = R[a];
            }
            if constexpr (H == 0) {
                static_assert(PK::rows() <= NP, "parking rows exceed the reserved block");
                double *PXw = sK + (2 * RP + 2 * (NP + 1) + NP) * 64;
#pragma unroll
                for (int m = 0; m < D; m++)
                    if (PK::need_x(m)) PXw[PK::row_x(m) * 64 + lane] = x[m];
#pragma unroll
                for (int t = 0; t < Model::NTAB; t++)
                    if (PK::need_t(t)) PXw[PK::row_t(t) * 64 + lane] = tv[t];
#pragma unroll
                for (int m = 0; m < D; m++)
                    if ((PK::rates() >> m) & 1u) {
                        PXw[PK::row_pm(m) * 64 + lane] = rpm[m];
                        PXw[(PK::row_pm(m) + 1) * 64 + lane] = rpp[m];
                    }
                if constexpr (PK::merged() != 0u) {
                    double qc = 0.0;
#pragma unroll
                    for (int m = 0; m < D; m++)
                        if (PM::mg(m)) { qc += rpm[m]; qc += rpp[m]; }
                    PXw[PK::row_q() * 64 + lane] = qc;
                }
            }
            pair_barrier();
        }
        FPP_STAMP(2)

        const int bck = A.bctype[K];
        const double *Gk = ro + A.core_off[K];
        auto partials = [&](int j, auto &&sink) __attribute__((always_inline)) -> double {
            double pv;
            if constexpr (K == 0) {
                double ah[RH];
#pragma unroll
                for (int i = 0; i < RH; i++) ah[i] = Gk[(size_t)j * RP + H * RH + i];
                double v = 0.0;
#pragma unroll
                for (int i = 0; i < RH; i++) v = fma(ah[i], sR[(H * RH + i) * 64 + lane], v);
                pv = v;
#pragma unroll
                for (int g = 0; g < NV; g++) sink(g, dot_reg<RH>(ah, Wh[g]));
            } else if constexpr (K == D - 1) {
                double ch[RH];
#pragma unroll
                for (int i = 0; i < RH; i++) ch[i] = Gk[(size_t)j * RP + H * RH + i];
                double v = 0.0;
#pragma unroll
                for (int i = 0; i < RH; i++) v = fma(sL[(H * RH + i) * 64 + lane], ch[i], v);
                pv = v;
#pragma unroll
                for (int g = 0; g < NV; g++) sink(g, dot_reg<RH>(Wh[g], ch));
            } else {
                const double *GC0 = Gk + (size_t)j * RP * RP;
                const double *GC = GC0 + (size_t)H * RH * RP;
                double ch[RH], ah[RH];
#pragma unroll
                for (int i = 0; i < RH; i++) { ch[i] = 0.0; ah[i] = 0.0; }
#pragma unroll
                for (int b = 0; b < RP; b++) {
                    const double rb = sR[b * 64 + lane];
#pragma unroll
// ... 414 lines not shown
```

### c3sc_amd/engine.py

```python
from __future__ import annotations

import ctypes as C
import os
from typing import Optional, Sequence

import numpy as np

_HERE = os.path.dirname(os.path.abspath(__file__))
LIB_PATH = os.path.join(_HERE, "csrc", "libc3sc_hip.so")
_LIB = None

c_double_p = C.POINTER(C.c_double)
c_size_p = C.POINTER(C.c_size_t)
c_int_p = C.POINTER(C.c_int)
c_i32_p = C.POINTER(C.c_int32)

EXPORTS = [
    "c3sc_hip_ctx_create", "c3sc_hip_ctx_destroy", "c3sc_hip_last_error", "c3sc_hip_device_count", "c3sc_hip_max_rank",
    "c3sc_hip_set_grid", "c3sc_hip_set_boundary", "c3sc_hip_set_consistent_ends", "c3sc_hip_get_consistent_ends", "c3sc_hip_cross_setup", "c3sc_hip_cross_iteration", "c3sc_hip_cross_iteration_streamed", "c3sc_hip_cross_wait_core", "c3sc_hip_cross_iteration_pi", "c3sc_hip_cross_confirm", "c3sc_hip_bellman_fibers_all", "c3sc_hip_policy_fibers_all", "c3sc_hip_cross_speculate", "c3sc_hip_comm_unique_id", "c3sc_hip_comm_create", "c3sc_hip_comm_destroy", "c3sc_hip_comm_world", "c3sc_hip_comm_rank", "c3sc_hip_comm_allgather", "c3sc_hip_cross_set_comm", "c3sc_hip_comm_exchange", "c3sc_hip_cross_options", "c3sc_hip_cross_grow_memo", "c3sc_hip_cross_fetch", "c3sc_hip_cross_free", "c3sc_hip_set_mca", "c3sc_hip_set_model",
    "c3sc_hip_set_controls", "c3sc_hip_upload_value", "c3sc_hip_upload_value_device", "c3sc_hip_set_variant",
    "c3sc_hip_bellman_fibers", "c3sc_hip_bellman_fibers_tables", "c3sc_hip_bellman_fibers_tables_host", "c3sc_hip_stencil_fibers", "c3sc_hip_bellman_fibers_host",
    "c3sc_hip_policy_fibers", "c3sc_hip_policy_fibers_host", "c3sc_hip_policy_fibers_tables", "c3sc_hip_policy_fibers_tables_host",
    "c3sc_hip_set_control_box", "c3sc_hip_bellman_fibers_box", "c3sc_hip_bellman_fibers_box_host", "c3sc_hip_policy_fibers_box",
    "c3sc_hip_policy_fibers_box_host",
    "c3sc_hip_stencil_fibers_host", "c3sc_hip_stencil_fibers_nb", "c3sc_hip_stencil_fibers_nb_host", "c3sc_hip_sync", "c3sc_hip_get_status", "c3sc_hip_last_kernel",
    "c3sc_hip_debug_read", "c3sc_hip_launch_count", "c3sc_hip_timer_start", "c3sc_hip_timer_stop", "c3sc_hip_peak_fma_f64", "c3sc_hip_peak_mfma_f64",
    "c3sc_hip_set_interp", "c3sc_hip_stencil_points", "c3sc_hip_simulate", "c3sc_hip_simulate_host", "c3sc_hip_normals",
    "c3sc_hip_integrate", "c3sc_hip_integrate_host",
    "c3sc_hip_model_compile", "c3sc_hip_model_code_object", "c3sc_hip_model_log",
    "c3sc_hip_set_game", "c3sc_hip_model_compile_ex", "c3sc_hip_model_code_object_ex",
    "c3sc_hip_model_compile_fh", "c3sc_hip_model_code_object_fh", "c3sc_hip_set_horizon_step", "c3sc_hip_upload_value_stack",
]

class SimArgs(C.Structure):
    _fields_ = [("n", C.c_size_t), ("d_x0", C.c_void_p), ("dt", C.c_double), ("nsteps", C.c_size_t),
                ("traj_offset", C.c_uint64), ("seed", C.c_uint64), ("d_noise", C.c_void_p), ("wrap_periodic", C.c_int),
                ("box", C.c_int), ("steps_per_launch", C.c_int), ("save_every", C.c_size_t), ("d_traj", C.c_void_p),
                ("d_u", C.c_void_p), ("d_cost", C.c_void_p), ("d_exit", C.c_void_p), ("d_vend", C.c_void_p),
                ("d_xfinal", C.c_void_p)]


ODE_FORWARD_EULER, ODE_RK4 = 0, 1
_ODE_METHODS = {"forward-euler": ODE_FORWARD_EULER, "euler": ODE_FORWARD_EULER, "rk4": ODE_RK4}


class OdeArgs(C.Structure):
    _fields_ = [("n", C.c_size_t), ("d_x0", C.c_void_p), ("dt_out", C.c_double), ("dt_int", C.c_double), ("nout", C.c_size_t),
                ("method", C.c_int), ("wrap_periodic", C.c_int), ("box", C.c_int), ("evals_per_launch", C.c_int),
                ("goal", C.c_void_p), ("keep", C.c_void_p), ("save_every", C.c_size_t), ("d_traj", C.c_void_p),
                ("d_u", C.c_void_p), ("d_cost", C.c_void_p), ("d_stop_step", C.c_void_p), ("d_stop_reason", C.c_void_p),
                ("d_vend", C.c_void_p), ("d_xfinal", C.c_void_p)]


class ModelSpec(C.Structure):
    _fields_ = [("source", C.c_char_p), ("name", C.c_char_p), ("d", C.c_int), ("du", C.c_int), ("udep_mask", C.c_uint),
                ("uconst_mask", C.c_uint), ("stage_udep", C.c_int), ("box", C.c_int), ("nranks", C.c_int),
                ("ranks", C.POINTER(C.c_int))]


class ModelSpecEx(C.Structure):
    _fields_ = [("base", ModelSpec), ("game", C.c_int)]


class ModelSpecFh(C.Structure):
    _fields_ = [("ex", ModelSpecEx), ("horizon", C.c_int)]


MODEL_USER = 1000
GAME_MINMAX, GAME_MAXMIN = 0, 1
_GAME_ORDERS = {"minmax": GAME_MINMAX, "upper": GAME_MINMAX, "maxmin": GAME_MAXMIN, "lower": GAME_MAXMIN}

VARIANT_AUTO, VARIANT_FIBER_PER_WAVE, VARIANT_FIBER_PER_LANE, VARIANT_FIBER_PAIR, VARIANT_FIBER_QUAD = 0, 1, 2, 3, 4


class C3scHipError(RuntimeError):
    pass


def load_library():
    global _LIB
    if _LIB is None:
        if not os.path.exists(LIB_PATH):
            raise C3scHipError(f"{LIB_PATH} is missing: build it with `python -c 'import __graft_entry__ as g; g.build()'` "
                               "or `make -C c3sc_amd/csrc`.  There is no CPU fallback.")
        import torch
        L = C.CDLL(LIB_PATH)
        L.c3sc_hip_last_error.restype = C.c_char_p
        L.c3sc_hip_last_error.argtypes = [C.c_void_p]
        L.c3sc_hip_last_kernel.restype = C.c_char_p
        L.c3sc_hip_last_kernel.argtypes = [C.c_void_p]
        L.c3sc_hip_ctx_destroy.restype = None
        L.c3sc_hip_ctx_destroy.argtypes = [C.c_void_p]
        L.c3sc_hip_bellman_fibers.argtypes = [C.c_void_p, C.c_int, C.c_size_t, C.c_void_p, C.c_void_p, C.c_void_p,
                                              C.c_void_p, C.c_void_p]
        L.c3sc_hip_stencil_fibers.argtypes = [C.c_void_p, C.c_int, C.c_size_t, C.c_void_p, C.c_void_p, C.c_void_p,
                                              C.c_void_p]
        L.c3sc_hip_bellman_fibers_host.argtypes = [C.c_void_p, C.c_int, C.c_size_t, C.c_void_p, C.c_void_p, C.c_void_p,
                                                   C.c_void_p]
        L.c3sc_hip_stencil_fibers_host.argtypes = [C.c_void_p, C.c_int, C.c_size_t, C.c_void_p, C.c_void_p, C.c_void_p]
        L.c3sc_hip_policy_fibers.argtypes = [C.c_void_p, C.c_int, C.c_size_t, C.c_void_p, C.c_void_p, C.c_void_p,
                                             C.c_void_p, C.c_void_p]
        L.c3sc_hip_policy_fibers_host.argtypes = [C.c_void_p, C.c_int, C.c_size_t, C.c_void_p, C.c_void_p, C.c_void_p,
                                                  C.c_void_p]
        L.c3sc_hip_stencil_fibers_nb_host.argtypes = [C.c_void_p, C.c_int, C.c_size_t, C.c_void_p, C.c_void_p, C.c_void_p,
                                                      C.c_void_p, C.c_void_p]
        L.c3sc_hip_bellman_fibers_tables_host.argtypes = [C.c_void_p, C.c_int, C.c_size_t] + [C.c_void_p] * 6
        L.c3sc_hip_policy_fibers_tables_host.argtypes = [C.c_void_p, C.c_int, C.c_size_t] + [C.c_void_p] * 6
        L.c3sc_hip_launch_count.restype = C.c_ulonglong
        L.c3sc_hip_sync.argtypes = [C.c_void_p, C.c_void_p]
        L.c3sc_hip_timer_start.argtypes = [C.c_void_p, C.c_void_p]
        L.c3sc_hip_timer_stop.argtypes = [C.c_void_p, C.c_void_p, C.POINTER(C.c_float)]
        L.c3sc_hip_upload_value_device.argtypes = [C.c_void_p, c_size_p, C.POINTER(C.c_void_p), C.c_void_p]
        L.c3sc_hip_cross_setup.argtypes = [C.c_void_p, c_size_p, C.POINTER(c_i32_p), C.POINTER(c_i32_p), C.c_int]
        L.c3sc_hip_cross_iteration.argtypes = [C.c_void_p, C.c_int, C.c_void_p]
        L.c3sc_hip_cross_confirm.argtypes = [C.c_void_p, c_int_p, C.c_void_p]
        L.c3sc_hip_cross_options.argtypes = [C.c_void_p, C.c_int, C.c_double]
        L.c3sc_hip_cross_iteration_pi.argtypes = [C.c_void_p, C.c_void_p, C.c_longlong, C.c_void_p]
        L.c3sc_hip_cross_grow_memo.argtypes = [C.c_void_p]
        L.c3sc_hip_cross_fetch.argtypes = [C.c_void_p, C.POINTER(c_double_p), C.POINTER(c_i32_p), C.POINTER(c_i32_p),
                                           C.POINTER(C.c_ulonglong), C.c_void_p]
        L.c3sc_hip_set_interp.argtypes = [C.c_void_p, C.c_int]
        L.c3sc_hip_stencil_points.argtypes = [C.c_void_p, C.c_size_t, C.c_void_p, C.c_void_p, C.c_void_p, C.c_void_p]
        L.c3sc_hip_simulate.argtypes = [C.c_void_p, C.POINTER(SimArgs), C.c_void_p]
        L.c3sc_hip_integrate.argtypes = [C.c_void_p, C.POINTER(OdeArgs), C.c_void_p]
        L.c3sc_hip_integrate_host.argtypes = [C.c_void_p, C.POINTER(OdeArgs)]
        L.c3sc_hip_normals.argtypes = [C.c_uint64, C.c_uint64, C.c_size_t, C.c_uint64, C.c_size_t, C.c_int, c_double_p]
        L.c3sc_hip_model_compile.argtypes = [C.POINTER(ModelSpec), c_int_p]
        L.c3sc_hip_model_code_object.argtypes = [C.POINTER(ModelSpec), C.c_void_p, c_size_p]
        L.c3sc_hip_model_log.restype = C.c_char_p
        L.c3sc_hip_model_log.argtypes = []
        L.c3sc_hip_model_compile_ex.argtypes = [C.POINTER(ModelSpecEx), c_int_p]
        L.c3sc_hip_model_code_object_ex.argtypes = [C.POINTER(ModelSpecEx), C.c_void_p, c_size_p]
        L.c3sc_hip_set_game.argtypes = [C.c_void_p, C.c_int, C.c_int, c_double_p, C.c_int, c_double_p, C.c_int]
        L.c3sc_hip_model_compile_fh.argtypes = [C.POINTER(ModelSpecFh), c_int_p]
        L.c3sc_hip_model_code_object_fh.argtypes = [C.POINTER(ModelSpecFh), C.c_void_p, c_size_p]
        L.c3sc_hip_set_horizon_step.argtypes = [C.c_void_p, C.c_double]
        L.c3sc_hip_upload_value_stack.argtypes = [C.c_void_p, C.c_int, c_size_p, C.POINTER(c_double_p)]
        _LIB = L
    return _LIB


def normals(seed: int, traj0: int, ntraj: int, step0: int, nsteps: int, dw: int) -> np.ndarray:
    L = load_library()
    out = np.empty((ntraj, nsteps, dw), dtype=np.float64)
    rc = L.c3sc_hip_normals(C.c_uint64(seed), C.c_uint64(traj0), C.c_size_t(ntraj), C.c_uint64(step0), C.c_size_t(nsteps),
                            C.c_int(dw), out.ctypes.data_as(c_double_p))
    if rc != 0:
        raise C3scHipError(f"c3sc_hip_normals failed (code {rc})")
    return out


def _model_spec(source, d, du, ranks, box, udep_mask, uconst_mask, stage_udep, name):
    rk = (C.c_int * max(1, len(ranks)))(*ranks)
    spec = ModelSpec(source.encode(), name.encode() if name is not None else None, int(d), int(du), int(udep_mask),
                     int(uconst_mask), 1 if stage_udep else 0, 1 if box else 0, len(ranks), rk if len(ranks) else None)
    spec._keep = rk
    return spec


def _model_fail(rc, what):
    log = load_library().c3sc_hip_model_log().decode(errors="replace")
    raise C3scHipError(f"{what} failed (code {rc}): {log}", rc)


def compile_model(source: str, d: int, du: int, ranks=(4, 8), box: bool = False, udep_mask: int = 0, uconst_mask: int = 0,
                  stage_udep: bool = True, name: Optional[str] = None, game: bool = False, horizon: bool = False) -> int:
    L = load_library()
    spec = _model_spec(source, d, du, tuple(ranks), box, udep_mask, uconst_mask, stage_udep, name)
    mid = C.c_int(0)
    if horizon:
        fh = ModelSpecFh(ModelSpecEx(spec, 1 if game else 0), 1)
        rc = L.c3sc_hip_model_compile_fh(C.byref(fh), C.byref(mid))
    elif game:
        ex = ModelSpecEx(spec, 1)
        rc = L.c3sc_hip_model_compile_ex(C.byref(ex), C.byref(mid))
    else:
        rc = L.c3sc_hip_model_compile(C.byref(spec), C.byref(mid))
    if rc != 0:
        _model_fail(rc, "c3sc_hip_model_compile")
    return mid.value


def code_object(source: str, d: int, du: int, ranks=(4, 8), box: bool = False, udep_mask: int = 0, uconst_mask: int = 0,
                stage_udep: bool = True, name: Optional[str] = None, game: bool = False, horizon: bool = False) -> bytes:
    L = load_library()
    spec = _model_spec(source, d, du, tuple(ranks), box, udep_mask, uconst_mask, stage_udep, name)
    cap = 16 << 20
    for _ in range(2):
        buf = C.create_string_buffer(cap)
        size = C.c_size_t(cap)
        if horizon:
            fh = ModelSpecFh(ModelSpecEx(spec, 1 if game else 0), 1)
            rc = L.c3sc_hip_model_code_object_fh(C.byref(fh), buf, C.byref(size))
        elif game:
            rc = L.c3sc_hip_model_code_object_ex(C.byref(ModelSpecEx(spec, 1)), buf, C.byref(size))
        else:
            rc = L.c3sc_hip_model_code_object(C.byref(spec), buf, C.byref(size))
        if rc == 0:
            return buf.raw[:size.value]
        if size.value <= cap:
            break
        cap = size.value
    _model_fail(rc, "c3sc_hip_model_code_object")


def game_split(index, nw: int):
    i = np.asarray(index)
    iu = np.where(i < 0, -1, i // nw)
    iw = np.where(i < 0, -1, i % nw)
    if np.ndim(index) == 0:
        return int(iu), int(iw)
    return iu, iw


def _f64(a):
    return np.ascontiguousarray(a, dtype=np.float64)


def _ptr_array(arrs):
    arr = (c_double_p * len(arrs))(*[a.ctypes.data_as(c_double_p) for a in arrs])
    arr._keep = arrs
    return arr


class BellmanEngine:

    def __init__(self, device: int = 0):
        self.L = load_library()
        h = C.c_void_p()
        rc = self.L.c3sc_hip_ctx_create(C.c_int(device), C.byref(h))
        if rc != 0:
            raise C3scHipError(f"c3sc_hip_ctx_create(device={device}) failed with code {rc} (no usable HIP device?)")
        self.h = h
        self.device = device
        self.w = None

    def close(self):
        if getattr(self, "h", None):
            self.L.c3sc_hip_ctx_destroy(self.h)
            self.h = None

    def __del__(self):
        try:
            self.close()
        except Exception:
            pass

    def _chk(self, rc, what):
        if rc != 0:
            msg = self.L.c3sc_hip_last_error(self.h)
            raise C3scHipError(f"{what} failed (code {rc}): {msg.decode() if msg else ''}")

    def set_grid(self, ngrid: Sequence[int], xgrid: Sequence[np.ndarray]):
        ng = np.ascontiguousarray(ngrid, dtype=np.uintp)
        xs = [_f64(g) for g in xgrid]
        self._chk(self.L.c3sc_hip_set_grid(self.h, C.c_int(len(ng)), ng.ctypes.data_as(c_size_p), _ptr_array(xs)),
                  "set_grid")
        self.ngrid = [int(n) for n in ngrid]
        self.d = len(self.ngrid)

    def set_boundary(self, bctype: Sequence[int], obstacles=()):
# ... 172 lines not shown
        if save_every > 0:
            res["traj"] = torch.empty((n, nsteps // save_every + 1, d), dtype=torch.float64, device=dev)
            res["u"] = torch.empty((n, (nsteps + save_every - 1) // save_every, du), dtype=torch.float64, device=dev)
            a.d_traj, a.d_u = res["traj"].data_ptr(), res["u"].data_ptr()
        a.d_cost, a.d_exit, a.d_vend, a.d_xfinal = (res["cost"].data_ptr(), res["exit"].data_ptr(), res["vend"].data_ptr(),
                                                    res["xfinal"].data_ptr())
        if stream_ptr is None:
            stream_ptr = torch.cuda.current_stream(dev).cuda_stream
        self._chk(self.L.c3sc_hip_simulate(self.h, C.byref(a), C.c_void_p(stream_ptr)), "simulate")
        return res

    def simulate_rc(self, args: "SimArgs", stream_ptr: int = 0) -> int:
        return int(self.L.c3sc_hip_simulate(self.h, C.byref(args), C.c_void_p(stream_ptr)))

    def integrate(self, x0_t, dt_out: float, nout: int, method: str = "rk4", dt_int: Optional[float] = None, goal=None,
                  keep_in=None, wrap_periodic: bool = False, box: bool = False, save_every: int = 0, evals_per_launch: int = 0,
                  stream_ptr: Optional[int] = None):
        import torch

        assert x0_t.is_cuda and x0_t.dtype == torch.float64 and x0_t.is_contiguous() and x0_t.shape[1] == self.d
        if method not in _ODE_METHODS:
            raise ValueError(f"integrate: unknown method {method!r} (forward-euler, rk4)")
        n, d, dev = x0_t.shape[0], self.d, x0_t.device
        du = getattr(self, "box_du", self.w.du) if box else self.w.du
        res = {"cost": torch.empty((n,), dtype=torch.float64, device=dev),
               "stop_step": torch.empty((n,), dtype=torch.int64, device=dev),
               "stop_reason": torch.empty((n,), dtype=torch.int32, device=dev),
               "vend": torch.empty((n,), dtype=torch.float64, device=dev),
               "xfinal": torch.empty((n, d), dtype=torch.float64, device=dev)}
        a = OdeArgs()
        a.n, a.d_x0, a.dt_out, a.nout = n, x0_t.data_ptr(), float(dt_out), int(nout)
        a.dt_int = 0.0 if dt_int is None else float(dt_int)
        a.method, a.wrap_periodic, a.box = _ODE_METHODS[method], int(bool(wrap_periodic)), int(bool(box))
        a.evals_per_launch, a.save_every = int(evals_per_launch), int(save_every)
        boxes = {}
        for key, b in (("goal", goal), ("keep", keep_in)):
            if b is not None:
                arr = np.ascontiguousarray(np.concatenate([np.asarray(b[0], dtype=np.float64).reshape(-1),
                                                           np.asarray(b[1], dtype=np.float64).reshape(-1)]))
                if arr.shape[0] != 2 * d:
                    raise ValueError(f"integrate: {key} needs (lo, hi) of {d} values each")
                boxes[key] = arr
                setattr(a, key, arr.ctypes.data)
        if save_every > 0:
            res["traj"] = torch.empty((n, nout // save_every + 1, d), dtype=torch.float64, device=dev)
            res["u"] = torch.empty((n, (nout + save_every - 1) // save_every, du), dtype=torch.float64, device=dev)
            a.d_traj, a.d_u = res["traj"].data_ptr(), res["u"].data_ptr()
        a.d_cost, a.d_stop_step, a.d_stop_reason = res["cost"].data_ptr(), res["stop_step"].data_ptr(), res["stop_reason"].data_ptr()
        a.d_vend, a.d_xfinal = res["vend"].data_ptr(), res["xfinal"].data_ptr()
        if stream_ptr is None:
            stream_ptr = torch.cuda.current_stream(dev).cuda_stream
        self._chk(self.L.c3sc_hip_integrate(self.h, C.byref(a), C.c_void_p(stream_ptr)), "integrate")
        return res

    def integrate_rc(self, args: "OdeArgs", stream_ptr: int = 0) -> int:
        return int(self.L.c3sc_hip_integrate(self.h, C.byref(args), C.c_void_p(stream_ptr)))

    def bellman_fibers_host(self, k: int, idx: np.ndarray, want_uidx=True, want_absorbed=True):
        idx = np.ascontiguousarray(idx, dtype=np.int32)
        F, N = idx.shape[0], self.ngrid[k]
        out = np.empty((F, N))
        ui = np.empty((F, N), dtype=np.int32) if want_uidx else None
        ab = np.empty((F, N), dtype=np.int32) if want_absorbed else None
        self._chk(self.L.c3sc_hip_bellman_fibers_host(self.h, k, F, idx.ctypes.data, out.ctypes.data,
                                                      ui.ctypes.data if ui is not None else None,
                                                      ab.ctypes.data if ab is not None else None), "bellman_fibers_host")
        return out, ui, ab

    def policy_fibers_host(self, k: int, idx: np.ndarray, policy: np.ndarray):
        idx = np.ascontiguousarray(idx, dtype=np.int32)
        policy = np.ascontiguousarray(policy, dtype=np.int32)
        F, N = idx.shape[0], self.ngrid[k]
        assert policy.shape == (F, N)
        out = np.empty((F, N))
        ab = np.empty((F, N), dtype=np.int32)
        self._chk(self.L.c3sc_hip_policy_fibers_host(self.h, k, F, idx.ctypes.data, policy.ctypes.data, out.ctypes.data,
                                                     ab.ctypes.data), "policy_fibers_host")
        return out, ab

    def set_control_box(self, lb, ub, grid=33, polish=2):
        lb, ub = _f64(lb), _f64(ub)
        self.box_du = len(lb)
        self._chk(self.L.c3sc_hip_set_control_box(self.h, len(lb), lb.ctypes.data_as(c_double_p), ub.ctypes.data_as(c_double_p),
                                                  int(grid), int(polish)), "set_control_box")

    def bellman_fibers_box_host(self, k: int, idx: np.ndarray):
        idx = np.ascontiguousarray(idx, dtype=np.int32)
        F, N = idx.shape[0], self.ngrid[k]
        out, uo, ab = np.empty((F, N)), np.empty((F, N, self.box_du)), np.empty((F, N), dtype=np.int32)
        self._chk(self.L.c3sc_hip_bellman_fibers_box_host(self.h, k, C.c_size_t(F), C.c_void_p(idx.ctypes.data), C.c_void_p(out.ctypes.data),
                                                          C.c_void_p(uo.ctypes.data), C.c_void_p(ab.ctypes.data)), "bellman_fibers_box_host")
        return out, uo, ab

    def policy_fibers_box_host(self, k: int, idx: np.ndarray, policy_u: np.ndarray):
        idx = np.ascontiguousarray(idx, dtype=np.int32)
        pu = _f64(policy_u)
        F, N = idx.shape[0], self.ngrid[k]
        out, ab = np.empty((F, N)), np.empty((F, N), dtype=np.int32)
        self._chk(self.L.c3sc_hip_policy_fibers_box_host(self.h, k, C.c_size_t(F), C.c_void_p(idx.ctypes.data), C.c_void_p(pu.ctypes.data),
                                                         C.c_void_p(out.ctypes.data), C.c_void_p(ab.ctypes.data)), "policy_fibers_box_host")
        return out, ab

    def bellman_fibers_tables_host(self, k: int, idx: np.ndarray, tables: np.ndarray, costs2: np.ndarray):
        idx = np.ascontiguousarray(idx, dtype=np.int32)
        tables = _f64(tables)
        costs2 = _f64(costs2)
        F, N = idx.shape[0], self.ngrid[k]
        out = np.empty((F, N))
        ui = np.empty((F, N), dtype=np.int32)
        ab = np.empty((F, N), dtype=np.int32)
        self._chk(self.L.c3sc_hip_bellman_fibers_tables_host(self.h, k, F, idx.ctypes.data, tables.ctypes.data,
                                                             costs2.ctypes.data, out.ctypes.data, ui.ctypes.data,
                                                             ab.ctypes.data), "bellman_fibers_tables_host")
        return out, ui, ab

    def policy_fibers_tables_host(self, k: int, idx: np.ndarray, tables: np.ndarray, costs2: np.ndarray, policy: np.ndarray):
        idx = np.ascontiguousarray(idx, dtype=np.int32)
        tables = _f64(tables)
        costs2 = _f64(costs2)
        policy = np.ascontiguousarray(policy, dtype=np.int32)
        F, N = idx.shape[0], self.ngrid[k]
        assert policy.shape == (F, N)
        out = np.empty((F, N))
        ab = np.empty((F, N), dtype=np.int32)
        self._chk(self.L.c3sc_hip_policy_fibers_tables_host(self.h, k, F, idx.ctypes.data, tables.ctypes.data, costs2.ctypes.data,
                                                            policy.ctypes.data, out.ctypes.data, ab.ctypes.data),
                  "policy_fibers_tables_host")
        return out, ab

    def stencil_fibers_host(self, k: int, idx: np.ndarray, nb_fixed=None, nb_vary=None):
        idx = np.ascontiguousarray(idx, dtype=np.int32)
        F, N = idx.shape[0], self.ngrid[k]
        costs = np.empty((F, N, 2 * self.d + 1))
        ab = np.empty((F, N), dtype=np.int32)
        nf = np.ascontiguousarray(nb_fixed, dtype=np.int32) if nb_fixed is not None else None
        nv = np.ascontiguousarray(nb_vary, dtype=np.int32) if nb_vary is not None else None
        self._chk(self.L.c3sc_hip_stencil_fibers_nb_host(self.h, k, F, idx.ctypes.data,
                                                         nf.ctypes.data if nf is not None else None,
                                                         nv.ctypes.data if nv is not None else None,
                                                         costs.ctypes.data, ab.ctypes.data), "stencil_fibers_nb_host")
        return costs, ab

    def sync(self, stream_ptr: int = 0):
        self._chk(self.L.c3sc_hip_sync(self.h, C.c_void_p(stream_ptr)), "sync")

    def status(self, clear=True) -> int:
        fl = C.c_uint(0)
        self._chk(self.L.c3sc_hip_get_status(self.h, C.byref(fl), C.c_int(1 if clear else 0)), "get_status")
        return fl.value

    def last_kernel(self) -> str:
        return self.L.c3sc_hip_last_kernel(self.h).decode()

    def timer_start(self, stream_ptr: int = 0):
        self._chk(self.L.c3sc_hip_timer_start(self.h, C.c_void_p(stream_ptr)), "timer_start")

    def timer_stop(self, stream_ptr: int = 0) -> float:
        ms = C.c_float(0)
        self._chk(self.L.c3sc_hip_timer_stop(self.h, C.c_void_p(stream_ptr), C.byref(ms)), "timer_stop")
        return ms.value

    def debug_read(self, n: int) -> np.ndarray:
        buf = np.zeros(n, dtype=np.uint64)
        self._chk(self.L.c3sc_hip_debug_read(self.h, C.c_void_p(buf.ctypes.data), C.c_size_t(n)), "debug_read")
        return buf

    def peak_fma_f64(self) -> float:
        v = C.c_double(0)
        self._chk(self.L.c3sc_hip_peak_fma_f64(self.h, C.byref(v)), "peak_fma_f64")
        return v.value

    def peak_mfma_f64(self) -> float:
        v = C.c_double(0)
        self._chk(self.L.c3sc_hip_peak_mfma_f64(self.h, C.byref(v)), "peak_mfma_f64")
        return v.value
```

### include/c3sc_hip.h

```cpp
#ifndef C3SC_HIP_H
#define C3SC_HIP_H

#ifndef __HIPCC_RTC__
#include <stddef.h>
#include <stdint.h>
#endif

#ifdef __cplusplus
extern "C" {
#endif

#define C3SC_MAX_DIM 12
#define C3SC_MAX_OBSTACLES 10
#define C3SC_MAX_PARAMS 8
#define C3SC_MAX_DU 4

enum {
    C3SC_OK = 0,
    C3SC_ERR_ARG = 1,
    C3SC_ERR_HIP = 2,
    C3SC_ERR_UNSUPPORTED = 3,
    C3SC_ERR_NODEVICE = 4
};

// ... 52 lines not shown
                               const int32_t *const *d_policy, double *const *d_out, int32_t *const *d_absorbed, void *stream);
int c3sc_hip_policy_fibers_host(c3sc_hip_ctx *ctx, int k, size_t F, const int32_t *h_idx, const int32_t *h_policy,
                                double *h_out, int32_t *h_absorbed);

int c3sc_hip_set_control_box(c3sc_hip_ctx *ctx, int du, const double *lb, const double *ub, int grid, int polish);
int c3sc_hip_bellman_fibers_box(c3sc_hip_ctx *ctx, int k, size_t F, const int32_t *d_idx, double *d_out, double *d_uopt,
                                int32_t *d_absorbed, void *stream);
int c3sc_hip_bellman_fibers_box_host(c3sc_hip_ctx *ctx, int k, size_t F, const int32_t *h_idx, double *h_out, double *h_uopt,
                                     int32_t *h_absorbed);
int c3sc_hip_policy_fibers_box(c3sc_hip_ctx *ctx, int k, size_t F, const int32_t *d_idx, const double *d_policy_u,
                               double *d_out, int32_t *d_absorbed, void *stream);
int c3sc_hip_policy_fibers_box_host(c3sc_hip_ctx *ctx, int k, size_t F, const int32_t *h_idx, const double *h_policy_u,
                                    double *h_out, int32_t *h_absorbed);

int c3sc_hip_bellman_fibers_tables(c3sc_hip_ctx *ctx, int k, size_t F, const int32_t *d_idx, const double *d_tables,
                                   const double *d_costs2, double *d_out, int32_t *d_uidx, int32_t *d_absorbed,
                                   void *stream);
int c3sc_hip_bellman_fibers_tables_host(c3sc_hip_ctx *ctx, int k, size_t F, const int32_t *h_idx,
                                        const double *h_tables, const double *h_costs2, double *h_out,
                                        int32_t *h_uidx, int32_t *h_absorbed);
int c3sc_hip_policy_fibers_tables(c3sc_hip_ctx *ctx, int k, size_t F, const int32_t *d_idx, const double *d_tables,
                                  const double *d_costs2, const int32_t *d_policy, double *d_out, int32_t *d_absorbed,
                                  void *stream);
int c3sc_hip_policy_fibers_tables_host(c3sc_hip_ctx *ctx, int k, size_t F, const int32_t *h_idx,
                                       const double *h_tables, const double *h_costs2, const int32_t *h_policy,
                                       double *h_out, int32_t *h_absorbed);

int c3sc_hip_stencil_fibers(c3sc_hip_ctx *ctx, int k, size_t F, const int32_t *d_idx, double *d_costs,
                            int32_t *d_absorbed, void *stream);

int c3sc_hip_stencil_fibers_nb(c3sc_hip_ctx *ctx, int k, size_t F, const int32_t *d_idx, const int32_t *d_nb_fixed,
                               const int32_t *d_nb_vary, double *d_costs, int32_t *d_absorbed, void *stream);
int c3sc_hip_stencil_fibers_nb_host(c3sc_hip_ctx *ctx, int k, size_t F, const int32_t *h_idx,
                                    const int32_t *h_nb_fixed, const int32_t *h_nb_vary, double *h_costs,
                                    int32_t *h_absorbed);

int c3sc_hip_bellman_fibers_host(c3sc_hip_ctx *ctx, int k, size_t F, const int32_t *h_idx, double *h_out,
                                 int32_t *h_uidx, int32_t *h_absorbed);
int c3sc_hip_stencil_fibers_host(c3sc_hip_ctx *ctx, int k, size_t F, const int32_t *h_idx, double *h_costs,
                                 int32_t *h_absorbed);

int c3sc_hip_set_interp(c3sc_hip_ctx *ctx, int constelm);
int c3sc_hip_stencil_points(c3sc_hip_ctx *ctx, size_t n, const double *d_x, double *d_out, int32_t *d_absorbed, void *stream);

typedef struct c3sc_hip_sim_args {
    size_t n;
    const double *d_x0;
    double dt;
    size_t nsteps;
    uint64_t traj_offset;
    uint64_t seed;
    const double *d_noise;
    int wrap_periodic;
    int box;
    int steps_per_launch;
    size_t save_every;
    double *d_traj;
    double *d_u;
    double *d_cost;
    int64_t *d_exit;
    double *d_vend;
    double *d_xfinal;
} c3sc_hip_sim_args;
int c3sc_hip_simulate(c3sc_hip_ctx *ctx, const c3sc_hip_sim_args *args, void *stream);
int c3sc_hip_simulate_host(c3sc_hip_ctx *ctx, const c3sc_hip_sim_args *args);

enum { C3SC_ODE_FORWARD_EULER = 0, C3SC_ODE_RK4 = 1 };
typedef struct c3sc_hip_ode_args {
    size_t n;
    const double *d_x0;
    double dt_out;
    double dt_int;
    size_t nout;
    int method;
    int wrap_periodic;
    int box;
    int evals_per_launch;
    const double *goal;
    const double *keep;
    size_t save_every;
    double *d_traj;
    double *d_u;
    double *d_cost;
    int64_t *d_stop_step;
    int32_t *d_stop_reason;
    double *d_vend;
    double *d_xfinal;
} c3sc_hip_ode_args;
int c3sc_hip_integrate(c3sc_hip_ctx *ctx, const c3sc_hip_ode_args *args, void *stream);
int c3sc_hip_integrate_host(c3sc_hip_ctx *ctx, const c3sc_hip_ode_args *args);
int c3sc_hip_normals(uint64_t seed, uint64_t traj0, size_t ntraj, uint64_t step0, size_t nsteps, int dw, double *out);

int c3sc_hip_cross_setup(c3sc_hip_ctx *ctx, const size_t *ranks, const int32_t *const *I, const int32_t *const *J, int new_sweep);
int c3sc_hip_cross_iteration(c3sc_hip_ctx *ctx, int box, void *stream);
int c3sc_hip_cross_iteration_streamed(c3sc_hip_ctx *ctx, int box, void *stream);
int c3sc_hip_cross_wait_core(c3sc_hip_ctx *ctx, int k, double *h_core);
int c3sc_hip_cross_confirm(c3sc_hip_ctx *ctx, int *confirmed, void *stream);
int c3sc_hip_cross_speculate(c3sc_hip_ctx *ctx, c3sc_hip_ctx *policy_ctx, long long policy_tag, int box, int *confirmed, void *stream);
int c3sc_hip_cross_iteration_pi(c3sc_hip_ctx *ctx, c3sc_hip_ctx *policy_ctx, long long policy_tag, void *stream);
int c3sc_hip_cross_options(c3sc_hip_ctx *ctx, int warm_pivots, double swap_tol);
int c3sc_hip_cross_grow_memo(c3sc_hip_ctx *ctx);
int c3sc_hip_cross_fetch(c3sc_hip_ctx *ctx, double *const *h_cores, int32_t *const *h_I, int32_t *const *h_J, unsigned long long *info,
                         void *stream);
void c3sc_hip_cross_free(c3sc_hip_ctx *ctx);

typedef struct c3sc_hip_comm c3sc_hip_comm;
int c3sc_hip_comm_unique_id(void *id128);
int c3sc_hip_comm_create(c3sc_hip_ctx *ctx, int world, int rank, const void *id128, c3sc_hip_comm **out);
void c3sc_hip_comm_destroy(c3sc_hip_comm *comm);
int c3sc_hip_comm_world(const c3sc_hip_comm *comm);
int c3sc_hip_comm_rank(const c3sc_hip_comm *comm);
int c3sc_hip_comm_allgather(c3sc_hip_comm *comm, const double *d_send, double *d_recv, size_t count, void *stream);
int c3sc_hip_cross_set_comm(c3sc_hip_ctx *ctx, c3sc_hip_comm *comm);
int c3sc_hip_comm_exchange(double *out, size_t F, size_t N, size_t lo, size_t hi, void *comm);

typedef struct c3sc_hip_model_spec {
    const char *source;
    const char *name;
    int d, du;
    unsigned udep_mask, uconst_mask;
    int stage_udep;
    int box;
    int nranks;
    const int *ranks;
} c3sc_hip_model_spec;
int c3sc_hip_model_compile(const c3sc_hip_model_spec *spec, int *model_id);
int c3sc_hip_model_code_object(const c3sc_hip_model_spec *spec, void *buf, size_t *size);
const char *c3sc_hip_model_log(void);

enum { C3SC_GAME_MINMAX = 0, C3SC_GAME_MAXMIN = 1 };
int c3sc_hip_set_game(c3sc_hip_ctx *ctx, int du_min, int nu, const double *U, int nw, const double *W, int order);
typedef struct c3sc_hip_model_spec_ex {
    c3sc_hip_model_spec base;
    int game;
} c3sc_hip_model_spec_ex;
int c3sc_hip_model_compile_ex(const c3sc_hip_model_spec_ex *spec, int *model_id);
int c3sc_hip_model_code_object_ex(const c3sc_hip_model_spec_ex *spec, void *buf, size_t *size);

typedef struct c3sc_hip_model_spec_fh {
    c3sc_hip_model_spec_ex ex;
    int horizon;
} c3sc_hip_model_spec_fh;
int c3sc_hip_model_compile_fh(const c3sc_hip_model_spec_fh *spec, int *model_id);
int c3sc_hip_model_code_object_fh(const c3sc_hip_model_spec_fh *spec, void *buf, size_t *size);
int c3sc_hip_set_horizon_step(c3sc_hip_ctx *ctx, double dt);
int c3sc_hip_upload_value_stack(c3sc_hip_ctx *ctx, int nstack, const size_t *ranks, const double *const *cores);

int c3sc_hip_sync(c3sc_hip_ctx *ctx, void *stream);
int c3sc_hip_get_status(c3sc_hip_ctx *ctx, unsigned *flags, int clear);
const char *c3sc_hip_last_kernel(const c3sc_hip_ctx *ctx);

int c3sc_hip_debug_read(c3sc_hip_ctx *ctx, unsigned long long *out, size_t n);
unsigned long long c3sc_hip_launch_count(void);

int c3sc_hip_timer_start(c3sc_hip_ctx *ctx, void *stream);
int c3sc_hip_timer_stop(c3sc_hip_ctx *ctx, void *stream, float *ms);

int c3sc_hip_peak_fma_f64(c3sc_hip_ctx *ctx, double *tflops);
int c3sc_hip_peak_mfma_f64(c3sc_hip_ctx *ctx, double *tflops);

#ifdef __cplusplus
}
#endif
#endif
```

Baseline: 32.44 billion.

## Group live fibers by major/minor grid key so waves share uniform core slices

Extends the fiber partition from a live/dead split into a multi-bin counting sort keyed on one or two grid coordinates. It uses per-block histograms, a column-parallel scan and a bitonic in-block sort for the scatter. The fiber-pair kernel gains a uniform path: when a wave's fibers share the same index on the grouped level, it reads that core slice through scalar loads (readfirstlane) instead of staging it into LDS. The aim is to cut LDS staging and barriers for those levels, at the cost of a heavier partition pass and more scratch memory. A debug API for reading back the last partition is also added.

```diff
diff --git a/c3sc_amd/csrc/c3sc_hip.hip b/c3sc_amd/csrc/c3sc_hip.hip
--- a/c3sc_amd/csrc/c3sc_hip.hip
+++ b/c3sc_amd/csrc/c3sc_hip.hip
@@ -891,6 +891,14 @@
     return v > 0 ? v : -1;
 }
 
+static long fiber_group_floor()
+{
+    const char *e = getenv("C3SC_FIBER_GROUP");
+    if (!e || !*e) return FPART_MIN_PER_BIN;
+    const long v = atol(e);
+    return v > 0 ? v : -1;
+}
+
 static int partition_fibers(c3sc_hip_ctx *c, const KernelEntry *e, const KArgs &A, LaunchIO &io, int slot, int &launched)
 {
     io.perm = nullptr;
@@ -901,20 +909,23 @@
     for (int m = 0; m < A.d; m++) faces = faces || (m != A.k && A.bctype[m] == C3SC_ABSORB);
     const long fmin = fiber_partition_min();
     if (!faces || fmin < 0 || A.F < fmin || A.F > 0x40000000L) return C3SC_OK;
-    const size_t need = fpart_bytes(A.F);
-    if (need > c->part_bytes[slot]) {
-        if (c->part[slot]) HIPCHK(c, hipFree(c->part[slot]));
-        c->part[slot] = nullptr;
-        c->part_bytes[slot] = 0;
-        HIPCHK(c, hipMalloc(&c->part[slot], need));
-        c->part_bytes[slot] = need;
-    }
-    const PartScratch ps = fpart_carve(c->part[slot], A.F);
     PartArgs P;
     P.d = A.d;
     P.k = A.k;
     P.F = A.F;
     for (int m = 0; m < MAXD; m++) { P.ngrid[m] = A.ngrid[m]; P.bctype[m] = A.bctype[m]; }
+    fpart_plan(P, fpp_group_levels(A.d, e->rp, A.k), fiber_group_floor());
+    const size_t need = fpart_bytes(A.F, P.nbins);
+    if (need > c->part_bytes[slot]) {
+        if (c->part[slot]) HIPCHK(c, hipFree(c->part[slot]));
+        c->part[slot] = nullptr;
+        c->part_bytes[slot] = 0;
+        c->part_last[slot] = {};
+        HIPCHK(c, hipMalloc(&c->part[slot], need));
+        c->part_bytes[slot] = need;
+    }
+    const PartScratch ps = fpart_carve(c->part[slot], A.F, P.nbins);
+    c->part_last[slot] = {ps.perm, ps.nlive, A.F, io.stream};
     HIPCHK(c, fpart_launch(P, io.idx, ps, io.stream));
     launched = 3;
     io.perm = ps.perm;
@@ -1613,6 +1624,24 @@
 
 unsigned long long c3sc_hip_launch_count(void) { return g_launches; }
 
+int c3sc_hip_last_partition(c3sc_hip_ctx *c, int slot, int32_t *perm, size_t cap, size_t *F, int *nlive)
+{
+    if (!c) return C3SC_ERR_ARG;
+    if (slot < 0 || slot > c3sc_hip_ctx::NSIDE || !F || !nlive) return fail(c, C3SC_ERR_ARG, "last_partition: bad arguments");
+    const auto &lp = c->part_last[slot];
+    if (!lp.perm) return fail(c, C3SC_ERR_ARG, "last_partition: no partition has run on this slot");
+    *F = (size_t)lp.F;
+    HIPCHK(c, hipStreamSynchronize(lp.stream));
+    int32_t nl = 0;
+    HIPCHK(c, hipMemcpy(&nl, lp.nlive, sizeof(nl), hipMemcpyDeviceToHost));
+    *nlive = nl;
+    if (perm) {
+        if (cap < (size_t)lp.F) return fail(c, C3SC_ERR_ARG, "last_partition: perm holds fewer than F entries");
+        HIPCHK(c, hipMemcpy(perm, lp.perm, (size_t)lp.F * sizeof(int32_t), hipMemcpyDeviceToHost));
+    }
+    return C3SC_OK;
+}
+
 int c3sc_hip_debug_read(c3sc_hip_ctx *c, unsigned long long *out, size_t n)
 {
     if (!c || !c->d_dbg || !out) return C3SC_ERR_ARG;
diff --git a/c3sc_amd/csrc/ctx.hpp b/c3sc_amd/csrc/ctx.hpp
--- a/c3sc_amd/csrc/ctx.hpp
+++ b/c3sc_amd/csrc/ctx.hpp
@@ -63,6 +63,11 @@
     hipEvent_t fork_ev = nullptr, join_ev[NSIDE] = {nullptr, nullptr};
     void *part[NSIDE + 1] = {nullptr, nullptr, nullptr};
     size_t part_bytes[NSIDE + 1] = {0, 0, 0};
+    struct {
+        int32_t *perm = nullptr, *nlive = nullptr;
+        long F = 0;
+        hipStream_t stream = nullptr;
+    } part_last[NSIDE + 1];
     void *scratch = nullptr;
     size_t scratch_bytes = 0;
     void *sim_state = nullptr;
diff --git a/c3sc_amd/csrc/fiber_partition.hpp b/c3sc_amd/csrc/fiber_partition.hpp
--- a/c3sc_amd/csrc/fiber_partition.hpp
+++ b/c3sc_amd/csrc/fiber_partition.hpp
@@ -6,38 +6,67 @@
 namespace c3sc {
 
 constexpr int FPART_THREADS = 256, FPART_PER_THREAD = 4, FPART_BLOCK = FPART_THREADS * FPART_PER_THREAD;
+static_assert(FPART_BLOCK == 1024, "the scatter packs (bin, position in the block) into one word with 10 position bits");
+constexpr int FPART_BIN_PER_THREAD = 8, FPART_MAX_BINS = FPART_THREADS * FPART_BIN_PER_THREAD;
+constexpr long FPART_MIN_PER_BIN = 128;
+constexpr int FPART_SCAN_BINS = 16;
 
 struct PartArgs {
     int d, k;
     long F;
     int ngrid[MAXD];
     int bctype[MAXD];
+    int kmaj = -1, kmin = -1;
+    int nmin = 1;
+    int nbins = 2;
 };
+
+inline void fpart_plan(PartArgs &P, KeyLevels kl, long floor)
+{
+    P.kmaj = P.kmin = -1;
+    P.nmin = 1;
+    P.nbins = 2;
+    if (floor < 0 || kl.n < 1) return;
+    const long nmaj = P.ngrid[kl.major];
+    if (nmaj + 1 > FPART_MAX_BINS || P.F < floor * nmaj) return;
+    P.kmaj = kl.major;
+    P.nbins = (int)nmaj + 1;
+    if (kl.n < 2) return;
+    const long nkeys = nmaj * P.ngrid[kl.minor];
+    if (nkeys + 1 > FPART_MAX_BINS || P.F < floor * nkeys) return;
+    P.kmin = kl.minor;
+    P.nmin = P.ngrid[kl.minor];
+    P.nbins = (int)nkeys + 1;
+}
 
 struct PartScratch {
     int32_t *perm = nullptr;
-    int32_t *blocks = nullptr;
+    int32_t *counts = nullptr;
+    int32_t *totals = nullptr;
     int32_t *nlive = nullptr;
-    uint8_t *flags = nullptr;
+    uint16_t *bins = nullptr;
 };
 
 __host__ __device__ constexpr size_t fpart_align(size_t b) { return (b + 255) & ~(size_t)255; }
 inline long fpart_blocks(long F) { return (F + FPART_BLOCK - 1) / FPART_BLOCK; }
-inline size_t fpart_bytes(long F)
-{
-    return fpart_align((size_t)F * 4) + fpart_align((size_t)fpart_blocks(F) * 4) + fpart_align(4) + fpart_align((size_t)F);
-}
-inline PartScratch fpart_carve(void *base, long F)
+inline size_t fpart_bytes(long F, int nbins)
+{
+    return fpart_align((size_t)F * 4) + fpart_align((size_t)fpart_blocks(F) * nbins * 4) + fpart_align((size_t)nbins * 4) + fpart_align(4) +
+           fpart_align((size_t)F * 2);
+}
+inline PartScratch fpart_carve(void *base, long F, int nbins)
 {
     PartScratch s;
     char *p = (char *)base;
     s.perm = (int32_t *)p;
     p += fpart_align((size_t)F * 4);
-    s.blocks = (int32_t *)p;
-    p += fpart_align((size_t)fpart_blocks(F) * 4);
+    s.counts = (int32_t *)p;
+    p += fpart_align((size_t)fpart_blocks(F) * nbins * 4);
+    s.totals = (int32_t *)p;
+    p += fpart_align((size_t)nbins * 4);
     s.nlive = (int32_t *)p;
     p += fpart_align(4);
-    s.flags = (uint8_t *)p;
+    s.bins = (uint16_t *)p;
     return s;
 }
 
@@ -75,60 +104,157 @@
     return before + inc - v;
 }
 
-__global__ void __launch_bounds__(FPART_THREADS) k_fpart_count(const PartArgs P, const int32_t *__restrict__ idx, uint8_t *__restrict__ flags,
-                                                               int32_t *__restrict__ blocks)
-{
-    const long f0 = (long)blockIdx.x * FPART_BLOCK + (long)threadIdx.x * FPART_PER_THREAD;
-    int live = 0;
-#pragma unroll
-    for (int i = 0; i < FPART_PER_THREAD; i++) {
-        const long f = f0 + i;
+__global__ void __launch_bounds__(FPART_THREADS) k_fpart_count(const PartArgs P, const int32_t *__restrict__ idx, uint16_t *__restrict__ bins,
+                                                               int32_t *__restrict__ counts)
+{
+    __shared__ int hist[FPART_MAX_BINS];
+    for (int b = threadIdx.x; b < P.nbins; b += FPART_THREADS) hist[b] = 0;
+    __syncthreads();
+    const long f0 = (long)blockIdx.x * FPART_BLOCK + threadIdx.x;
+#pragma unroll
+    for (int i = 0; i < FPART_PER_THREAD; i++) {
+        const long f = f0 + (long)i * FPART_THREADS;
         if (f < P.F) {
-            const bool dead = fiber_dead(P, idx, f);
-            flags[f] = dead ? 1 : 0;
-            live += dead ? 0 : 1;
-        }
-    }
-    int total;
-    (void)fpart_block_scan(live, total);
-    if (threadIdx.x == 0) blocks[blockIdx.x] = total;
-}
-
-__global__ void __launch_bounds__(FPART_THREADS) k_fpart_scan(int32_t *__restrict__ blocks, long nblocks, int32_t *__restrict__ nlive)
-{
-    int carry = 0;
-    for (long b0 = 0; b0 < nblocks; b0 += FPART_THREADS) {
-        const long b = b0 + threadIdx.x;
-        const int v = b < nblocks ? blocks[b] : 0;
+            int bin = P.nbins - 1;
+            if (!fiber_dead(P, idx, f)) {
+                bin = P.kmaj >= 0 ? idx[f * P.d + P.kmaj] : 0;
+                if (P.kmin >= 0) bin = bin * P.nmin + idx[f * P.d + P.kmin];
+                bin = min(max(bin, 0), P.nbins - 2);
+            }
+            bins[f] = (uint16_t)bin;
+            atomicAdd(&hist[bin], 1);
+        }
+    }
+    __syncthreads();
+    int32_t *row = counts + (size_t)blockIdx.x * P.nbins;
+    for (int b = threadIdx.x; b < P.nbins; b += FPART_THREADS) row[b] = hist[b];
+}
+
+constexpr int FPART_SCAN_THREADS = 1024, FPART_SCAN_CHUNK = 8;
+__global__ void __launch_bounds__(FPART_SCAN_THREADS) k_fpart_scan(int32_t *__restrict__ counts, long nblocks, int nbins, int32_t *__restrict__ totals)
+{
+    constexpr int NS = FPART_SCAN_THREADS / FPART_SCAN_BINS;
+    __shared__ int part[NS][FPART_SCAN_BINS];
+    const int c = threadIdx.x % FPART_SCAN_BINS, s = threadIdx.x / FPART_SCAN_BINS;
+    const int bin = blockIdx.x * FPART_SCAN_BINS + c;
+    const bool on = bin < nbins;
+    const long per = (nblocks + NS - 1) / NS, b0 = s * per < nblocks ? s * per : nblocks, b1 = b0 + per < nblocks ? b0 + per : nblocks;
+    int sum = 0;
+    if (on)
+        for (long b = b0; b < b1; b += FPART_SCAN_CHUNK) {
+            int v[FPART_SCAN_CHUNK];
+#pragma unroll
+            for (int q = 0; q < FPART_SCAN_CHUNK; q++) v[q] = b + q < b1 ? counts[(size_t)(b + q) * nbins + bin] : 0;
+#pragma unroll
+            for (int q = 0; q < FPART_SCAN_CHUNK; q++) sum += v[q];
+        }
+    part[s][c] = sum;
+    __syncthreads();
+    int run = 0, total = 0;
+    for (int q = 0; q < NS; q++) {
+        const int v = part[q][c];
+        if (q < s) run += v;
+        total += v;
+    }
+    if (on) {
+        for (long b = b0; b < b1; b += FPART_SCAN_CHUNK) {
+            int v[FPART_SCAN_CHUNK];
+#pragma unroll
+            for (int q = 0; q < FPART_SCAN_CHUNK; q++) v[q] = b + q < b1 ? counts[(size_t)(b + q) * nbins + bin] : 0;
+#pragma unroll
+            for (int q = 0; q < FPART_SCAN_CHUNK; q++) {
+                if (b + q < b1) counts[(size_t)(b + q) * nbins + bin] = run;
+                run += v[q];
+            }
+        }
+        if (s == 0) totals[bin] = total;
+    }
+}
+
+__global__ void __launch_bounds__(FPART_THREADS) k_fpart_scatter(long F, int nbins, const uint16_t *__restrict__ bins, const int32_t *__restrict__ counts,
+                                                                 const int32_t *__restrict__ totals, int32_t *__restrict__ nlive,
+                                                                 int32_t *__restrict__ perm)
+{
+    __shared__ int base[FPART_MAX_BINS];
+    __shared__ int start[FPART_MAX_BINS];
+    __shared__ unsigned srt[FPART_BLOCK];
+    const int tid = threadIdx.x;
+    {
+        int v[FPART_BIN_PER_THREAD], sum = 0;
+#pragma unroll
+        for (int i = 0; i < FPART_BIN_PER_THREAD; i++) {
+            const int b = tid * FPART_BIN_PER_THREAD + i;
+            v[i] = b < nbins ? totals[b] : 0;
+            sum += v[i];
+        }
         int total;
-        const int ex = fpart_block_scan(v, total);
-        if (b < nblocks) blocks[b] = carry + ex;
-        carry += total;
-    }
-    if (threadIdx.x == 0) *nlive = carry;
-}
-
-__global__ void __launch_bounds__(FPART_THREADS) k_fpart_scatter(long F, const uint8_t *__restrict__ flags, const int32_t *__restrict__ blocks,
-                                                                 const int32_t *__restrict__ nlive, int32_t *__restrict__ perm)
-{
-    const long fb = (long)blockIdx.x * FPART_BLOCK, f0 = fb + (long)threadIdx.x * FPART_PER_THREAD;
-    bool dead[FPART_PER_THREAD];
-    int live = 0;
-#pragma unroll
-    for (int i = 0; i < FPART_PER_THREAD; i++) {
-        dead[i] = (f0 + i < F) ? flags[f0 + i] != 0 : true;
-        live += dead[i] ? 0 : 1;
-    }
-    int total;
-    const int ex = fpart_block_scan(live, total);
-    const long live_before = blocks[blockIdx.x];
-    long lpos = live_before + ex;
-    long dpos = (long)*nlive + (fb - live_before) + ((long)threadIdx.x * FPART_PER_THREAD - ex);
-#pragma unroll
-    for (int i = 0; i < FPART_PER_THREAD; i++) {
-        if (f0 + i < F) {
-            if (dead[i]) perm[dpos++] = (int32_t)(f0 + i);
-            else perm[lpos++] = (int32_t)(f0 + i);
+        int ex = fpart_block_scan(sum, total);
+#pragma unroll
+        for (int i = 0; i < FPART_BIN_PER_THREAD; i++) {
+            base[tid * FPART_BIN_PER_THREAD + i] = ex;
+            ex += v[i];
+        }
+    }
+    const long fb = (long)blockIdx.x * FPART_BLOCK;
+    if (nbins == 2) {
+        if (blockIdx.x == 0 && tid == 0) *nlive = base[1];
+        bool dead[FPART_PER_THREAD];
+        int live = 0;
+#pragma unroll
+        for (int i = 0; i < FPART_PER_THREAD; i++) {
+            const long f = fb + tid * FPART_PER_THREAD + i;
+            dead[i] = f < F ? bins[f] != 0 : true;
+            live += dead[i] ? 0 : 1;
+        }
+        int total;
+        const int ex = fpart_block_scan(live, total);
+        const int32_t *row = counts + (size_t)blockIdx.x * 2;
+        long lpos = (long)row[0] + ex, dpos = (long)base[1] + row[1] + (tid * FPART_PER_THREAD - ex);
+#pragma unroll
+        for (int i = 0; i < FPART_PER_THREAD; i++) {
+            const long f = fb + tid * FPART_PER_THREAD + i;
+            if (f < F) {
+                if (dead[i]) perm[dpos++] = (int32_t)f;
+                else perm[lpos++] = (int32_t)f;
+            }
+        }
+        return;
+    }
+#pragma unroll
+    for (int i = 0; i < FPART_PER_THREAD; i++) {
+        const int p = tid * FPART_PER_THREAD + i;
+        srt[p] = fb + p < F ? ((unsigned)bins[fb + p] << 10) | (unsigned)p : 0xffffffffu;
+    }
+    for (int k = 2; k <= FPART_BLOCK; k <<= 1)
+        for (int j = k >> 1; j > 0; j >>= 1) {
+            __syncthreads();
+#pragma unroll
+            for (int e = tid; e < FPART_BLOCK / 2; e += FPART_THREADS) {
+                const int lo = ((e & ~(j - 1)) << 1) | (e & (j - 1)), hi = lo | j;
+                const unsigned a = srt[lo], b = srt[hi];
+                const bool up = (lo & k) == 0;
+                if ((a > b) == up) {
+                    srt[lo] = b;
+                    srt[hi] = a;
+                }
+            }
+        }
+    __syncthreads();
+    if (blockIdx.x == 0 && tid == 0) *nlive = base[nbins - 1];
+    unsigned w[FPART_PER_THREAD];
+#pragma unroll
+    for (int i = 0; i < FPART_PER_THREAD; i++) {
+        const int s = tid * FPART_PER_THREAD + i;
+        w[i] = srt[s];
+        if (w[i] != 0xffffffffu && (s == 0 || (srt[s - 1] >> 10) != (w[i] >> 10))) start[w[i] >> 10] = s;
+    }
+    __syncthreads();
+    const int32_t *row = counts + (size_t)blockIdx.x * nbins;
+#pragma unroll
+    for (int i = 0; i < FPART_PER_THREAD; i++) {
+        if (w[i] != 0xffffffffu) {
+            const int s = tid * FPART_PER_THREAD + i, bin = (int)(w[i] >> 10);
+            perm[(long)base[bin] + row[bin] + (s - start[bin])] = (int32_t)(fb + (w[i] & 1023u));
         }
     }
 }
@@ -136,10 +262,11 @@
 inline hipError_t fpart_launch(const PartArgs &P, const int32_t *idx, const PartScratch &s, hipStream_t stream)
 {
     const long nb = fpart_blocks(P.F);
-    hipLaunchKernelGGL(k_fpart_count, dim3((unsigned)nb), dim3(FPART_THREADS), 0, stream, P, idx, s.flags, s.blocks);
-    hipLaunchKernelGGL(k_fpart_scan, dim3(1), dim3(FPART_THREADS), 0, stream, s.blocks, nb, s.nlive);
-    hipLaunchKernelGGL(k_fpart_scatter, dim3((unsigned)nb), dim3(FPART_THREADS), 0, stream, P.F, (const uint8_t *)s.flags, (const int32_t *)s.blocks,
-                       (const int32_t *)s.nlive, s.perm);
+    hipLaunchKernelGGL(k_fpart_count, dim3((unsigned)nb), dim3(FPART_THREADS), 0, stream, P, idx, s.bins, s.counts);
+    hipLaunchKernelGGL(k_fpart_scan, dim3((unsigned)((P.nbins + FPART_SCAN_BINS - 1) / FPART_SCAN_BINS)), dim3(FPART_SCAN_THREADS), 0, stream, s.counts, nb,
+                       P.nbins, s.totals);
+    hipLaunchKernelGGL(k_fpart_scatter, dim3((unsigned)nb), dim3(FPART_THREADS), 0, stream, P.F, P.nbins, (const uint16_t *)s.bins,
+                       (const int32_t *)s.counts, (const int32_t *)s.totals, s.nlive, s.perm);
     return hipGetLastError();
 }
 
diff --git a/c3sc_amd/csrc/fold_lds.hpp b/c3sc_amd/csrc/fold_lds.hpp
--- a/c3sc_amd/csrc/fold_lds.hpp
+++ b/c3sc_amd/csrc/fold_lds.hpp
@@ -103,6 +103,64 @@
     }
 }
 
+template <int RP, int NV, bool ROWVEC>
+__device__ __forceinline__ void apply_uni(const double *__restrict__ G, double (&v)[NV][RP])
+{
+    constexpr int NE = RP * RP, NB = (NE + 3) / 4;
+    double t[NV][RP];
+#pragma unroll
+    for (int s = 0; s < NV; s++)
+#pragma unroll
+        for (int i = 0; i < RP; i++) t[s][i] = 0.0;
+#pragma unroll
+    for (int b0 = 0; b0 < NE; b0 += NB) {
+        double g[NB];
+#pragma unroll
+        for (int e = 0; e < NB; e++) g[e] = (b0 + e < NE) ? G[b0 + e] : 0.0;
+        __builtin_amdgcn_sched_barrier(0);
+#pragma unroll
+        for (int e = 0; e < NB; e++) asm volatile("" : "+s"(g[e]));
+#pragma unroll
+        for (int e = 0; e < NB; e++) {
+            if (b0 + e < NE) {
+                const int a = (b0 + e) % RP, b = (b0 + e) / RP;
+#pragma unroll
+                for (int s = 0; s < NV; s++) {
+                    if constexpr (ROWVEC) t[s][b] = fma(v[s][a], g[e], t[s][b]);
+                    else t[s][a] = fma(g[e], v[s][b], t[s][a]);
+                }
+            }
+        }
+#pragma unroll
+        for (int s = 0; s < NV; s++)
+#pragma unroll
+            for (int i = 0; i < RP; i++) pin(t[s][i]);
+    }
+#pragma unroll
+    for (int s = 0; s < NV; s++)
+#pragma unroll
+        for (int i = 0; i < RP; i++) v[s][i] = t[s][i];
+}
+
+template <int RP, int NW, int FIRST, int COUNT, bool ROWVEC, int NVMAX>
+__device__ __forceinline__ void apply_range_uni(const double *__restrict__ G, double (&W)[NW][RP])
+{
+    if constexpr (COUNT > 0) {
+        constexpr int NV = COUNT >= NVMAX ? NVMAX : COUNT;
+        double tmp[NV][RP];
+#pragma unroll
+        for (int s = 0; s < NV; s++)
+#pragma unroll
+            for (int a = 0; a < RP; a++) tmp[s][a] = W[FIRST + s][a];
+        apply_uni<RP, NV, ROWVEC>(G, tmp);
+#pragma unroll
+        for (int s = 0; s < NV; s++)
+#pragma unroll
+            for (int a = 0; a < RP; a++) W[FIRST + s][a] = tmp[s][a];
+        apply_range_uni<RP, NW, FIRST + NV, COUNT - NV, ROWVEC, NVMAX>(G, W);
+    }
+}
+
 template <int RP>
 __device__ inline double dot_reg(const double (&a)[RP], const double (&b)[RP])
 {
diff --git a/c3sc_amd/csrc/kernel_common.hpp b/c3sc_amd/csrc/kernel_common.hpp
--- a/c3sc_amd/csrc/kernel_common.hpp
+++ b/c3sc_amd/csrc/kernel_common.hpp
@@ -74,6 +74,35 @@
 __host__ __device__ inline long pair_tabL_off(const KArgs &A, int rp) { return A.pair_img_off[A.d - 1] + pair_img_doubles(A.ngrid[A.d - 1], rp); }
 __host__ __device__ inline long pair_tabR_off(const KArgs &A, int rp) { return pair_tabL_off(A, rp) + pair_tab_doubles(A.ngrid[0], A.ngrid[1], rp); }
 
+struct KeyLevels {
+    int n, major, minor;
+};
+__host__ __device__ constexpr KeyLevels fpp_key_levels(int d, int k, bool tab)
+{
+    const int lfirst = (tab && k >= 2) ? 2 : 1, rfirst = (tab && k <= d - 3) ? d - 3 : d - 2;
+    const int nl = k - lfirst > 0 ? k - lfirst : 0, nr = rfirst - k > 0 ? rfirst - k : 0;
+    if (nl > 0 && nr > 0) return {2, k - 1, k + 1};
+    if (nl > 0) return {nl > 1 ? 2 : 1, k - 1, nl > 1 ? k - 2 : -1};
+    if (nr > 0) return {nr > 1 ? 2 : 1, k + 1, nr > 1 ? k + 2 : -1};
+    return {0, -1, -1};
+}
+#ifndef FPP_DIRECT_MAXD
+#define FPP_DIRECT_MAXD 3
+#endif
+#ifndef FPP_EDGE_TABLES
+#define FPP_EDGE_TABLES 1
+#endif
+#ifndef FPP_GROUP_FOLD
+#define FPP_GROUP_FOLD 1
+#endif
+__host__ __device__ constexpr bool fpp_group_fold_optout(int d, int rp, int k) { return d == 7 && rp == 10 && k == 1; }
+__host__ __device__ constexpr KeyLevels fpp_group_levels(int d, int rp, int k)
+{
+    const bool direct = d <= FPP_DIRECT_MAXD && rp <= 8;
+    if (!FPP_GROUP_FOLD || direct || fpp_group_fold_optout(d, rp, k)) return {0, -1, -1};
+    return fpp_key_levels(d, k, FPP_EDGE_TABLES && d >= 4);
+}
+
 __device__ inline int game_list_to_pair(const KArgs &A, int p)
 {
     return A.game_order == C3SC_GAME_MAXMIN ? (p % A.game_gsz) * A.game_ngrp + p / A.game_gsz : p;
diff --git a/c3sc_amd/csrc/kernel_fiber_pair.hpp b/c3sc_amd/csrc/kernel_fiber_pair.hpp
--- a/c3sc_amd/csrc/kernel_fiber_pair.hpp
+++ b/c3sc_amd/csrc/kernel_fiber_pair.hpp
@@ -72,6 +72,38 @@
 #pragma unroll
         for (int a = 0; a < RP; a++) W[FIRST + s][a] = tmp[s + 1][a];
     apply_core<RP, NW, FIRST + N1, COUNT - N1, ROWVEC, FPP_NV>(G, W);
+}
+
+template <int RP, int NW, int FIRST, int COUNT, bool ROWVEC>
+__device__ __forceinline__ void apply_uni_and(const double *__restrict__ G, double (&W)[NW][RP], double (&E)[RP])
+{
+    constexpr int N1 = COUNT >= FPP_NV - 1 ? FPP_NV - 1 : COUNT;
+    double tmp[N1 + 1][RP];
+#pragma unroll
+    for (int a = 0; a < RP; a++) tmp[0][a] = E[a];
+#pragma unroll
+    for (int s = 0; s < N1; s++)
+#pragma unroll
+        for (int a = 0; a < RP; a++) tmp[s + 1][a] = W[FIRST + s][a];
+    apply_uni<RP, N1 + 1, ROWVEC>(G, tmp);
+#pragma unroll
+    for (int a = 0; a < RP; a++) E[a] = tmp[0][a];
+#pragma unroll
+    for (int s = 0; s < N1; s++)
+#pragma unroll
+        for (int a = 0; a < RP; a++) W[FIRST + s][a] = tmp[s + 1][a];
+    apply_range_uni<RP, NW, FIRST + N1, COUNT - N1, ROWVEC, FPP_NV>(G, W);
+}
+
+template <bool KEY, class Body>
+__device__ __forceinline__ void fold_level(int v, Body &&body)
+{
+    if constexpr (KEY) {
+        const int u = __builtin_amdgcn_readfirstlane(v);
+        if (__ballot(v != u) == 0ull) body(std::true_type{}, u);
+        else body(std::false_type{}, 0);
+    } else
+        body(std::false_type{}, 0);
 }
 
 __device__ inline void pair_barrier()
@@ -238,6 +270,16 @@
         p.products = ls + rs;
         for (int it = 0; it < NIT; it++) p.products += cost(it);
         return p;
+    }
+    __host__ __device__ static constexpr int level_products(int m)
+    {
+        return 3 + (m < K ? left_before<0>(m) + left_before<1>(m) : right_after<0>(m) + right_after<1>(m));
+    }
+    __host__ __device__ static constexpr int uniform_rounds() { return fpp_key_levels(D, K, TAB).n; }
+    __host__ __device__ static constexpr int uniform_products()
+    {
+        constexpr KeyLevels kl = fpp_key_levels(D, K, TAB);
+        return (kl.n > 0 ? level_products(kl.major) : 0) + (kl.n > 1 ? level_products(kl.minor) : 0);
     }
     __host__ __device__ static constexpr int owner(int it)
     {
@@ -337,6 +379,9 @@
     constexpr int NOWN = (NOL + NOR) > 0 ? (NOL + NOR) : 1;
     constexpr int NP = NV + 1;
     constexpr bool DIRECT = fpp_direct<Model, RP>();
+    constexpr KeyLevels KL = fpp_group_levels(D, RP, K);
+    constexpr bool GROUP = PART && KL.n > 0;
+    static_assert(!GROUP || fpp_key_levels(D, K, ET).major == KL.major, "the key levels follow the kernel's own fold plan");
     static_assert(RP % 2 == 0, "rank-split kernel needs an even padded rank");
     const int lane = threadIdx.x & 63;
     const int N = A.N;
@@ -485,53 +530,62 @@
             }
             auto left_step = [&](auto mc) __attribute__((always_inline)) {
                 constexpr int m = decltype(mc)::value;
-                constexpr int str = DIRECT ? RP * RP : fpl_lds_stride(RP * RP);
-                constexpr int before = PM::template left_before<H>(m);
-                constexpr bool PAIR = !PM::mg(m) && PM::owner(m) == H, ACC = PM::mg(m) && PM::owner(PM::UL) == H;
-                double nw[RP];
-                const double *src = sK;
-                FPP_STAMP(1)
-                if constexpr (DIRECT) src = ro + A.core_off[m];
-                else {
-                    pair_barrier();
-                    stage_core_image<H>(sK, A.img_base + A.pair_img_off[m], A.ngrid[m] * str);
-                    pair_barrier();
-                }
-                if constexpr (PM::ltab() && m == PL.lfirst) left_combine();
-                FPP_STAMP(7)
-                const double *G = src + fi[m] * str;
-                if constexpr (PAIR || ACC) {
-                    double t0[1][RP], t1[1][RP];
-#pragma unroll
-                    for (int a = 0; a < RP; a++) { t0[0][a] = L[a]; t1[0][a] = L[a]; }
+                auto body = [&](auto uc, int iu) __attribute__((always_inline)) {
+                    constexpr bool UNI = decltype(uc)::value;
+                    constexpr int str = (DIRECT || UNI) ? RP * RP : fpl_lds_stride(RP * RP);
+                    constexpr int before = PM::template left_before<H>(m);
+                    constexpr bool PAIR = !PM::mg(m) && PM::owner(m) == H, ACC = PM::mg(m) && PM::owner(PM::UL) == H;
+                    double nw[RP];
+                    const double *src = sK;
+                    FPP_STAMP(1)
+                    if constexpr (DIRECT || UNI) src = ro + A.core_off[m];
+                    else {
+                        pair_barrier();
+                        stage_core_image<H>(sK, A.img_base + A.pair_img_off[m], A.ngrid[m] * str);
+                        pair_barrier();
+                    }
+                    if constexpr (PM::ltab() && m == PL.lfirst) left_combine();
+                    FPP_STAMP(7)
+                    const double *G = src + (UNI ? iu : fi[m]) * str;
+                    if constexpr (PAIR || ACC) {
+                        double t0[1][RP], t1[1][RP];
+#pragma unroll
+                        for (int a = 0; a < RP; a++) { t0[0][a] = L[a]; t1[0][a] = L[a]; }
+                        if constexpr (DIRECT) {
+                            apply_glb<RP, 1, true>(src + nbm[m] * str, t0);
+                            apply_glb<RP, 1, true>(src + nbp[m] * str, t1);
+                        } else if constexpr (UNI) {
+                            apply_uni<RP, 1, true>(src + __builtin_amdgcn_readfirstlane(nbm[m]) * str, t0);
+                            apply_uni<RP, 1, true>(src + __builtin_amdgcn_readfirstlane(nbp[m]) * str, t1);
+                        } else {
+                            vecmat_lds<RP, 1>(src + nbm[m] * str, t0);
+                            vecmat_lds<RP, 1>(src + nbp[m] * str, t1);
+                        }
+#pragma unroll
+                        for (int a = 0; a < RP; a++) {
+                            if constexpr (PAIR) { W[before][a] = t0[0][a]; W[before + 1][a] = t1[0][a]; }
+                            else nw[a] = fma(rpp[m], t1[0][a], rpm[m] * t0[0][a]);
+                        }
+                    }
                     if constexpr (DIRECT) {
-                        apply_glb<RP, 1, true>(src + nbm[m] * str, t0);
-                        apply_glb<RP, 1, true>(src + nbp[m] * str, t1);
-                    } else {
-                        vecmat_lds<RP, 1>(src + nbm[m] * str, t0);
-                        vecmat_lds<RP, 1>(src + nbp[m] * str, t1);
-                    }
-#pragma unroll
-                    for (int a = 0; a < RP; a++) {
-                        if constexpr (PAIR) { W[before][a] = t0[0][a]; W[before + 1][a] = t1[0][a]; }
-                        else nw[a] = fma(rpp[m], t1[0][a], rpm[m] * t0[0][a]);
-                    }
-                }
-                if constexpr (DIRECT) {
-                    double tl[1][RP];
-#pragma unroll
-                    for (int a = 0; a < RP; a++) tl[0][a] = L[a];
-                    apply_glb<RP, 1, true>(G, tl);
-#pragma unroll
-                    for (int a = 0; a < RP; a++) L[a] = tl[0][a];
-                    apply_range_glb<RP, NOWN, 0, before, true>(G, W);
-                } else
-                    apply_core_and<RP, NOWN, 0, before, true>(G, W, L);
-                if constexpr (ACC) {
-                    constexpr int su = PM::template lslot<H>(PM::UL);
-#pragma unroll
-                    for (int a = 0; a < RP; a++) W[su][a] = (m == PM::first_l()) ? nw[a] : W[su][a] + nw[a];
-                }
+                        double tl[1][RP];
+#pragma unroll
+                        for (int a = 0; a < RP; a++) tl[0][a] = L[a];
+                        apply_glb<RP, 1, true>(G, tl);
+#pragma unroll
+                        for (int a = 0; a < RP; a++) L[a] = tl[0][a];
+                        apply_range_glb<RP, NOWN, 0, before, true>(G, W);
+                    } else if constexpr (UNI)
+                        apply_uni_and<RP, NOWN, 0, before, true>(G, W, L);
+                    else
+                        apply_core_and<RP, NOWN, 0, before, true>(G, W, L);
+                    if constexpr (ACC) {
+                        constexpr int su = PM::template lslot<H>(PM::UL);
+#pragma unroll
+                        for (int a = 0; a < RP; a++) W[su][a] = (m == PM::first_l()) ? nw[a] : W[su][a] + nw[a];
+                    }
+                };
+                fold_level<GROUP && (m == KL.major || (KL.n > 1 && m == KL.minor))>(fi[m], body);
             };
             [&]<int... Ms>(std::integer_sequence<int, Ms...>) { (left_step(std::integral_constant<int, Ms + PL.lfirst>{}), ...); }
             (std::make_integer_sequence<int, (K > PL.lfirst ? K - PL.lfirst : 0)>{});
@@ -602,53 +656,62 @@
             }
             auto right_step = [&](auto mc) __attribute__((always_inline)) {
                 constexpr int m = decltype(mc)::value;
-                constexpr int str = DIRECT ? RP * RP : fpl_lds_stride(RP * RP);
-                constexpr int after = PM::template right_after<H>(m);
-                constexpr bool PAIR = !PM::mg(m) && PM::owner(m) == H, ACC = PM::mg(m) && PM::owner(PM::UR) == H;
-                double nw[RP];
-                const double *src = sK;
-                FPP_STAMP(1)
-                if constexpr (DIRECT) src = ro + A.core_off[m];
-                else {
-                    pair_barrier();
-                    stage_core_image<H>(sK, A.img_base + A.pair_img_off[m], A.ngrid[m] * str);
-                    pair_barrier();
-                }
-                if constexpr (PM::rtab() && m == PL.rfirst) right_combine();
-                FPP_STAMP(7)
-                const double *G = src + fi[m] * str;
-                if constexpr (PAIR || ACC) {
-                    double t0[1][RP], t1[1][RP];
-#pragma unroll
-                    for (int a = 0; a < RP; a++) { t0[0][a] = R[a]; t1[0][a] = R[a]; }
+                auto body = [&](auto uc, int iu) __attribute__((always_inline)) {
+                    constexpr bool UNI = decltype(uc)::value;
+                    constexpr int str = (DIRECT || UNI) ? RP * RP : fpl_lds_stride(RP * RP);
+                    constexpr int after = PM::template right_after<H>(m);
+                    constexpr bool PAIR = !PM::mg(m) && PM::owner(m) == H, ACC = PM::mg(m) && PM::owner(PM::UR) == H;
+                    double nw[RP];
+                    const double *src = sK;
+                    FPP_STAMP(1)
+                    if constexpr (DIRECT || UNI) src = ro + A.core_off[m];
+                    else {
+                        pair_barrier();
+                        stage_core_image<H>(sK, A.img_base + A.pair_img_off[m], A.ngrid[m] * str);
+                        pair_barrier();
+                    }
+                    if constexpr (PM::rtab() && m == PL.rfirst) right_combine();
+                    FPP_STAMP(7)
+                    const double *G = src + (UNI ? iu : fi[m]) * str;
+                    if constexpr (PAIR || ACC) {
+                        double t0[1][RP], t1[1][RP];
+#pragma unroll
+                        for (int a = 0; a < RP; a++) { t0[0][a] = R[a]; t1[0][a] = R[a]; }
+                        if constexpr (DIRECT) {
+                            apply_glb<RP, 1, false>(src + nbm[m] * str, t0);
+                            apply_glb<RP, 1, false>(src + nbp[m] * str, t1);
+                        } else if constexpr (UNI) {
+                            apply_uni<RP, 1, false>(src + __builtin_amdgcn_readfirstlane(nbm[m]) * str, t0);
+                            apply_uni<RP, 1, false>(src + __builtin_amdgcn_readfirstlane(nbp[m]) * str, t1);
+                        } else {
+                            matvec_lds<RP, 1>(src + nbm[m] * str, t0);
+                            matvec_lds<RP, 1>(src + nbp[m] * str, t1);
+                        }
+#pragma unroll
+                        for (int a = 0; a < RP; a++) {
+                            if constexpr (PAIR) { W[NOL + after][a] = t0[0][a]; W[NOL + after + 1][a] = t1[0][a]; }
+                            else nw[a] = fma(rpp[m], t1[0][a], rpm[m] * t0[0][a]);
+                        }
+                    }
                     if constexpr (DIRECT) {
-                        apply_glb<RP, 1, false>(src + nbm[m] * str, t0);
-                        apply_glb<RP, 1, false>(src + nbp[m] * str, t1);
-                    } else {
-                        matvec_lds<RP, 1>(src + nbm[m] * str, t0);
-                        matvec_lds<RP, 1>(src + nbp[m] * str, t1);
-                    }
-#pragma unroll
-                    for (int a = 0; a < RP; a++) {
-                        if constexpr (PAIR) { W[NOL + after][a] = t0[0][a]; W[NOL + after + 1][a] = t1[0][a]; }
-                        else nw[a] = fma(rpp[m], t1[0][a], rpm[m] * t0[0][a]);
-                    }
-                }
-                if constexpr (DIRECT) {
-                    double tr[1][RP];
-#pragma unroll
-                    for (int a = 0; a < RP; a++) tr[0][a] = R[a];
-                    apply_glb<RP, 1, false>(G, tr);
-#pragma unroll
-                    for (int a = 0; a < RP; a++) R[a] = tr[0][a];
-                    apply_range_glb<RP, NOWN, NOL, after, false>(G, W);
-                } else
-                    apply_core_and<RP, NOWN, NOL, after, false>(G, W, R);
-                if constexpr (ACC) {
-                    constexpr int su = PM::template lslot<H>(PM::UR);
-#pragma unroll
-                    for (int a = 0; a < RP; a++) W[su][a] = (m == PM::first_r()) ? nw[a] : W[su][a] + nw[a];
-                }
+                        double tr[1][RP];
+#pragma unroll
+                        for (int a = 0; a < RP; a++) tr[0][a] = R[a];
+                        apply_glb<RP, 1, false>(G, tr);
+#pragma unroll
+                        for (int a = 0; a < RP; a++) R[a] = tr[0][a];
+                        apply_range_glb<RP, NOWN, NOL, after, false>(G, W);
+                    } else if constexpr (UNI)
+                        apply_uni_and<RP, NOWN, NOL, after, false>(G, W, R);
+                    else
+                        apply_core_and<RP, NOWN, NOL, after, false>(G, W, R);
+                    if constexpr (ACC) {
+                        constexpr int su = PM::template lslot<H>(PM::UR);
+#pragma unroll
+                        for (int a = 0; a < RP; a++) W[su][a] = (m == PM::first_r()) ? nw[a] : W[su][a] + nw[a];
+                    }
+                };
+                fold_level<GROUP && (m == KL.major || (KL.n > 1 && m == KL.minor))>(fi[m], body);
             };
             [&]<int... Ms>(std::integer_sequence<int, Ms...>) { (right_step(std::integral_constant<int, PL.rfirst - Ms>{}), ...); }
             (std::make_integer_sequence<int, (PL.rfirst - K > 0 ? PL.rfirst - K : 0)>{});
diff --git a/c3sc_amd/engine.py b/c3sc_amd/engine.py
--- a/c3sc_amd/engine.py
+++ b/c3sc_amd/engine.py
@@ -24,7 +24,7 @@
     "c3sc_hip_set_control_box", "c3sc_hip_bellman_fibers_box", "c3sc_hip_bellman_fibers_box_host", "c3sc_hip_policy_fibers_box",
     "c3sc_hip_policy_fibers_box_host",
     "c3sc_hip_stencil_fibers_host", "c3sc_hip_stencil_fibers_nb", "c3sc_hip_stencil_fibers_nb_host", "c3sc_hip_sync", "c3sc_hip_get_status", "c3sc_hip_last_kernel",
-    "c3sc_hip_debug_read", "c3sc_hip_launch_count", "c3sc_hip_timer_start", "c3sc_hip_timer_stop", "c3sc_hip_peak_fma_f64", "c3sc_hip_peak_mfma_f64",
+    "c3sc_hip_debug_read", "c3sc_hip_launch_count", "c3sc_hip_last_partition", "c3sc_hip_timer_start", "c3sc_hip_timer_stop", "c3sc_hip_peak_fma_f64", "c3sc_hip_peak_mfma_f64",
     "c3sc_hip_set_interp", "c3sc_hip_stencil_points", "c3sc_hip_simulate", "c3sc_hip_simulate_host", "c3sc_hip_normals",
     "c3sc_hip_integrate", "c3sc_hip_integrate_host",
     "c3sc_hip_model_compile", "c3sc_hip_model_code_object", "c3sc_hip_model_log",
@@ -107,6 +107,7 @@
         L.c3sc_hip_bellman_fibers_tables_host.argtypes = [C.c_void_p, C.c_int, C.c_size_t] + [C.c_void_p] * 6
         L.c3sc_hip_policy_fibers_tables_host.argtypes = [C.c_void_p, C.c_int, C.c_size_t] + [C.c_void_p] * 6
         L.c3sc_hip_launch_count.restype = C.c_ulonglong
+        L.c3sc_hip_last_partition.argtypes = [C.c_void_p, C.c_int, C.c_void_p, C.c_size_t, C.POINTER(C.c_size_t), C.POINTER(C.c_int)]
         L.c3sc_hip_sync.argtypes = [C.c_void_p, C.c_void_p]
         L.c3sc_hip_timer_start.argtypes = [C.c_void_p, C.c_void_p]
         L.c3sc_hip_timer_stop.argtypes = [C.c_void_p, C.c_void_p, C.POINTER(C.c_float)]
@@ -585,6 +586,14 @@
     def last_kernel(self) -> str:
         return self.L.c3sc_hip_last_kernel(self.h).decode()
 
+    def last_partition(self, slot: int = 0):
+        F, nl = C.c_size_t(0), C.c_int(0)
+        self._chk(self.L.c3sc_hip_last_partition(self.h, slot, None, 0, C.byref(F), C.byref(nl)), "last_partition")
+        perm = np.empty(F.value, dtype=np.int32)
+        self._chk(self.L.c3sc_hip_last_partition(self.h, slot, perm.ctypes.data_as(C.c_void_p), perm.size, C.byref(F), C.byref(nl)),
+                  "last_partition")
+        return perm, nl.value
+
     def timer_start(self, stream_ptr: int = 0):
         self._chk(self.L.c3sc_hip_timer_start(self.h, C.c_void_p(stream_ptr)), "timer_start")
 
diff --git a/include/c3sc_hip.h b/include/c3sc_hip.h
--- a/include/c3sc_hip.h
+++ b/include/c3sc_hip.h
@@ -228,6 +228,7 @@
 
 int c3sc_hip_debug_read(c3sc_hip_ctx *ctx, unsigned long long *out, size_t n);
 unsigned long long c3sc_hip_launch_count(void);
+int c3sc_hip_last_partition(c3sc_hip_ctx *ctx, int slot, int32_t *perm, size_t cap, size_t *F, int *nlive);
 
 int c3sc_hip_timer_start(c3sc_hip_ctx *ctx, void *stream);
 int c3sc_hip_timer_stop(c3sc_hip_ctx *ctx, void *stream, float *ms);
```

Result: faster. 34.16 billion, median of 6 (+5.3%).
